# SonSang/dmesh_renderer

Measured on AMD Instinct MI355X. Metric: fwd+bwd Mpixels/sec @1080p, 500k tris; grad max-abs-err vs ref, higher is better.
Workload: dtype f32

## Files before the change

dmesh_renderer_amd/csrc/dmr_api.hip:

```cpp
#include <algorithm>
#include <atomic>
#include <chrono>
#include <cstdio>
#include <cstdlib>
#include <cstring>
#include <functional>
#include <map>
#include <mutex>
#include <string>
#include <vector>

#include "dmr_kernels.hpp"

namespace {

thread_local std::string g_err;

int fail(const std::string& m) { g_err = m; return 1; }

#define DMR_HIP(expr)                                                                           \
    do {                                                                                        \
        hipError_t e_ = (expr);                                                                 \
        if (e_ != hipSuccess) return fail(std::string(#expr) + ": " + hipGetErrorString(e_));   \
    } while (0)

constexpr size_t ALIGN = 256;
inline size_t up(size_t n) { return (n + ALIGN - 1) & ~(ALIGN - 1); }

struct Carver {
    char* base; size_t off;
    explicit Carver(void* b) : base(reinterpret_cast<char*>(b)), off(0) {}
    template <class T> T* take(size_t count) {
        T* p = base ? reinterpret_cast<T*>(base + off) : nullptr;
        off += up(count * sizeof(T));
        return p;
    }
};

struct PointState { float4* vproj; };
struct FaceState { uint2* rect; float* key_depth; float* max_depth; uint32_t* tiles_touched; void* facerec; void* colrec; void* tetrec; };
struct ImageState {
    uint32_t* tile_count; uint32_t* tile_offset; uint32_t* tile_cursor; int* num_rendered;
    float* final_T; float* final_prev_T; uint32_t* n_contrib;
    uint32_t* tile_hits; uint32_t* tile_bound; uint32_t* scan_tmp; uint32_t* hit_offset; uint32_t* tile_used; unsigned long long* hit_total; uint32_t* tile_order;
    int32_t* first_face; int32_t* first_tet; int32_t* last_face; int32_t* last_tet; uint8_t* is_active;
    float* mats;
    int* seed;
    unsigned long long* mask_offset;
    dmr::TetSeq* seq;
};
struct BinningState {
    uint64_t* keys; uint32_t* face_list; uint32_t capacity; unsigned long long mask_offset, mask_first;
    char* base; unsigned long long seq_offset; uint32_t seq_steps;
};

size_t carve_point(void* b, size_t BP, PointState& s) { Carver c(b); s.vproj = c.take<float4>(BP); return c.off; }
size_t carve_face(void* b, size_t BF, size_t F, size_t T, bool tet, FaceState& s) {
    Carver c(b);
    s.rect = c.take<uint2>(BF); s.key_depth = c.take<float>(BF);
    s.max_depth = tet ? c.take<float>(BF) : nullptr;
    s.tiles_touched = c.take<uint32_t>(BF);
    s.facerec = s.colrec = s.tetrec = nullptr;
    if (tet) {
        s.facerec = c.take<char>(F * dmr::tet_facerec_bytes());
        s.colrec = c.take<char>(F * dmr::tet_colrec_bytes());
        s.tetrec = c.take<char>(T * dmr::tet_tetrec_bytes());
    }
    return c.off;
}
size_t carve_image(void* b, size_t B, size_t ntiles, size_t npix, bool tet, ImageState& s) {
    Carver c(b);
    s.mats = c.take<float>(64 * B);
    s.seed = c.take<int>(1);
    s.mask_offset = c.take<unsigned long long>(2);
    s.tile_count = c.take<uint32_t>(ntiles); s.tile_hits = c.take<uint32_t>(ntiles); s.tile_bound = c.take<uint32_t>(ntiles);
    s.scan_tmp = c.take<uint32_t>(dmr::scan_tmp_words((int)ntiles));
    s.hit_offset = c.take<uint32_t>(ntiles + 1); s.tile_used = c.take<uint32_t>(ntiles); s.hit_total = c.take<unsigned long long>(1);
    s.tile_offset = c.take<uint32_t>(ntiles + 1);
    s.tile_cursor = c.take<uint32_t>(ntiles); s.num_rendered = c.take<int>(1);
    s.tile_order = c.take<uint32_t>(ntiles);
    s.final_T = c.take<float>(npix); s.final_prev_T = c.take<float>(npix); s.n_contrib = c.take<uint32_t>(npix);
    if (tet) {
        s.first_face = c.take<int32_t>(npix); s.first_tet = c.take<int32_t>(npix);
        s.last_face = c.take<int32_t>(npix); s.last_tet = c.take<int32_t>(npix);
        s.is_active = c.take<uint8_t>(npix);
        s.seq = c.take<dmr::TetSeq>(1);
    } else {
        s.first_face = s.first_tet = s.last_face = s.last_tet = nullptr; s.is_active = nullptr;
        s.seq = nullptr;
    }
    return c.off;
}
size_t carve_binning(void* b, size_t R, size_t mask_tiles, size_t seq_tiles, size_t seq_steps, BinningState& s) {
    Carver c(b);
    s.face_list = c.take<uint32_t>(R); s.keys = c.take<uint64_t>(R);
    s.capacity = (uint32_t)std::min<size_t>(R, 0xffffffffu);
    s.mask_offset = c.off;
    s.mask_first = dmr::mask_first_slots(R, mask_tiles);
    if (mask_tiles && R > 0) c.take<uint4>(dmr::mask_slots(R, mask_tiles) * 256);
    s.base = reinterpret_cast<char*>(b); s.seq_offset = c.off; s.seq_steps = (uint32_t)seq_steps;
    if (seq_steps) c.take<char>(dmr::tet_seq_bytes(seq_tiles, seq_steps));
    return c.off;
}

struct Dims { int gx, gy, r0, r1, ntiles; size_t BP, BF, npix; };

dmr_scene canonical(const dmr_scene* s, const float* mats) {
    dmr_scene c = *s;
    const size_t n = 16 * (size_t)s->B;
    c.mv_mats = mats; c.proj_mats = mats + n; c.inv_mv_mats = mats + 2 * n; c.inv_proj_mats = mats + 3 * n;
    c.mats_transposed = 0;
    return c;
}

int check_scene(const dmr_scene* s, bool tet, Dims& d) {
    if (!s) return fail("null scene");
    if (s->B <= 0 || s->W <= 0 || s->H <= 0 || s->P < 0 || s->F < 0 || s->T < 0) return fail("bad dimensions");
    if ((int64_t)s->B * s->P > INT32_MAX || (int64_t)s->B * s->F > INT32_MAX || (int64_t)s->B * s->W * s->H > INT32_MAX)
        return fail("problem too large for 32-bit indexing");
    d.gx = (s->W + dmr::TILE - 1) / dmr::TILE;
    d.gy = (s->H + dmr::TILE - 1) / dmr::TILE;
    if (d.gx > 65535 || d.gy > 65535) return fail("image too large (tile coordinates must fit 16 bits)");
    d.r0 = s->row_begin; d.r1 = s->row_end;
    if (d.r0 == 0 && d.r1 == 0) d.r1 = d.gy;
    d.r0 = std::max(0, std::min(d.gy, d.r0));
    d.r1 = std::max(d.r0, std::min(d.gy, d.r1));
    d.ntiles = s->B * d.gx * d.gy;
    d.BP = (size_t)s->B * s->P; d.BF = (size_t)s->B * s->F; d.npix = (size_t)s->B * s->W * s->H;
    if (tet && s->F > 0 && s->P > 0 && (!s->tets || !s->face_tets || !s->tet_faces)) return fail("tet topology missing");
    if (tet && s->F >= (1 << 28)) return fail("too many faces for the tet renderer (face ids must fit 28 bits)");
    return 0;
}

struct SizeRead {
    void* slot = nullptr; uint32_t seq = 0;
    volatile unsigned long long* word(int which) const { return reinterpret_cast<volatile unsigned long long*>(slot) + which; }
    uint32_t next_seq() { seq = (seq + 1u) & 0xffffffu; if (seq == 0u) seq = 1u; return seq; }
};
SizeRead* size_read() {
    thread_local std::map<int, SizeRead> per_device;
    int dev = 0;
    if (hipGetDevice(&dev) != hipSuccess) return nullptr;
    SizeRead& sr = per_device[dev];
    if (!sr.slot) {
        if (hipHostMalloc(&sr.slot, 64, hipHostMallocCoherent | hipHostMallocPortable) != hipSuccess) { sr.slot = nullptr; return nullptr; }
        memset(sr.slot, 0, 64);
    }
    return &sr;
}
int wait_size(volatile unsigned long long* w, uint32_t seq, hipStream_t st, unsigned long long* size) {
    const auto t0 = std::chrono::steady_clock::now();
    for (uint32_t spins = 0;; spins++) {
        const unsigned long long v = *w;
        if ((uint32_t)(v >> 40) == (seq & 0xffffffu)) { std::atomic_thread_fence(std::memory_order_acquire); *size = v & ((1ull << 40) - 1ull); return 0; }
        if ((spins & 1023u) == 1023u && std::chrono::steady_clock::now() - t0 > std::chrono::milliseconds(50)) break;
#if defined(__x86_64__) || defined(__i386__)
        __builtin_ia32_pause();
#endif
    }
    DMR_HIP(hipStreamSynchronize(st));
    const unsigned long long v = *w;
    if ((uint32_t)(v >> 40) != (seq & 0xffffffu)) return fail("the size word was not written (internal error)");
    *size = v & ((1ull << 40) - 1ull);
    return 0;
}

std::mutex g_overflow_mu;
std::map<int, uint32_t*> g_overflow;
uint32_t* overflow_word(int dev, bool create) {
    std::lock_guard<std::mutex> lk(g_overflow_mu);
    auto it = g_overflow.find(dev);
    if (it != g_overflow.end()) return it->second;
    if (!create) return nullptr;
    void* p = nullptr;
    if (hipHostMalloc(&p, 64, hipHostMallocCoherent | hipHostMallocPortable) != hipSuccess) return nullptr;
    *reinterpret_cast<volatile uint32_t*>(p) = 0u;
    return g_overflow[dev] = reinterpret_cast<uint32_t*>(p);
}

bool stream_is_capturing(hipStream_t st) {
    hipStreamCaptureStatus cs = hipStreamCaptureStatusNone;
    if (hipStreamIsCapturing(st, &cs) != hipSuccess) { (void)hipGetLastError(); return false; }
    return cs != hipStreamCaptureStatusNone;
}

struct SizeKey {
    int v[7];
    bool operator<(const SizeKey& o) const { return memcmp(v, o.v, sizeof(v)) < 0; }
};
struct SizeGuess { double rendered_per_face = 0.0, hits_per_face = 0.0; uint32_t* seq_steps = nullptr; };
std::mutex g_size_mu;
std::map<SizeKey, SizeGuess> g_size_cache;
std::atomic<uint64_t> g_redo_count{0};
int size_bucket(size_t BF) { int b = 0; while ((BF >> (b + 1)) != 0) b++; return b; }
SizeKey size_key(const dmr_scene* s, bool tet, const Dims& d) {
    return SizeKey{{s->B, s->W, s->H, d.r0, d.r1, tet ? 1 : 0, size_bucket(d.BF)}};
}
double lookup_estimate(const SizeKey& key, double SizeGuess::* field) {
    for (int db : {0, -1, 1}) {
        SizeKey k = key; k.v[6] += db;
        auto it = g_size_cache.find(k);
        if (it != g_size_cache.end() && it->second.*field > 0.0) return it->second.*field;
    }
    return 0.0;
}
uint64_t padded(uint64_t n) { return n + n / 4 + 4096; }

int run_forward(const dmr_scene* s, bool tet, const Dims& d, dmr_alloc_fn alloc, void* ctx, hipStream_t st,
                PointState& ps, FaceState& fs, ImageState& is, int* num_rendered,
                const std::function<void(const BinningState&)>& render) {
    PointState tp; FaceState tf; ImageState ti;
    void* pb = alloc(ctx, DMR_BUF_POINT, carve_point(nullptr, d.BP, tp));
    void* fb = alloc(ctx, DMR_BUF_FACE, carve_face(nullptr, d.BF, (size_t)s->F, (size_t)s->T, tet, tf));
    void* ib = alloc(ctx, DMR_BUF_IMAGE, carve_image(nullptr, (size_t)s->B, (size_t)d.ntiles, d.npix, tet, ti));
    if (!pb || !fb || !ib) return fail("scratch allocation failed");
    carve_point(pb, d.BP, ps);
    carve_face(fb, d.BF, (size_t)s->F, (size_t)s->T, tet, fs);
    carve_image(ib, (size_t)s->B, (size_t)d.ntiles, d.npix, tet, is);
    const bool async = (s->flags & DMR_FLAG_ASYNC) != 0 || stream_is_capturing(st);
    int dev = 0;
    DMR_HIP(hipGetDevice(&dev));
    uint32_t* overflow = overflow_word(dev, !async);

    auto front = [&](unsigned long long* host_R, uint32_t host_seq, uint64_t capacity, uint32_t* ovf) -> int {
        dmr::launch_project_verts(*s, ps.vproj, is.mats, is.tile_count, (size_t)(is.scan_tmp + dmr::SCAN_TMP_BUCKETS - is.tile_count), st);
        dmr::launch_setup_faces(*s, tet, ps.vproj, d.gx, d.gy, d.r0, d.r1, fs.rect, fs.key_depth, fs.max_depth,
                                fs.tiles_touched, is.tile_count, st);
        dmr::launch_scan_tiles(d.ntiles, is.tile_count, is.tile_offset, is.tile_cursor, is.num_rendered, host_R, host_seq, is.tile_order,
                               is.scan_tmp, (uint32_t)std::min<uint64_t>(capacity, 0xffffffffu), ovf, st);
        return 0;
    };
    size_t seq_steps = 0;
    if (tet) {
        std::lock_guard<std::mutex> lk(g_size_mu);
        SizeGuess& g = g_size_cache[size_key(s, tet, d)];
        if (!g.seq_steps && !async) {
            void* w = nullptr;
            if (hipHostMalloc(&w, 64, hipHostMallocCoherent | hipHostMallocPortable) == hipSuccess) {
                g.seq_steps = reinterpret_cast<uint32_t*>(w);
                *reinterpret_cast<volatile uint32_t*>(g.seq_steps) = 0u;
            } else (void)hipGetLastError();
        }
        if (g.seq_steps) {
            const uint64_t longest = *reinterpret_cast<volatile uint32_t*>(g.seq_steps);
            if (longest) {
                const uint64_t budget = 16ull << 30;
                const uint64_t per4 = dmr::tet_seq_bytes((size_t)d.ntiles, 4);
                seq_steps = (size_t)(std::min<uint64_t>((longest + longest / 4 + 4 + 3) / 4, std::max<uint64_t>(budget / std::max<uint64_t>(per4, 1), 1)) * 4);
            }
        }
    }
    auto rest = [&](uint64_t capacity) -> int {
        BinningState tb, bs;
        const size_t mask_tiles = tet ? 0 : (size_t)d.ntiles;
        void* bb = alloc(ctx, DMR_BUF_BINNING, carve_binning(nullptr, (size_t)capacity, mask_tiles, (size_t)d.ntiles, seq_steps, tb));
        if (!bb && (capacity > 0 || seq_steps > 0)) return fail("binning allocation failed");
        carve_binning(bb, (size_t)capacity, mask_tiles, (size_t)d.ntiles, seq_steps, bs);

        if (capacity > 0) {
            dmr::launch_scatter_faces(*s, d.gx, d.gy, fs.rect, fs.key_depth, fs.tiles_touched, is.tile_cursor, bs.keys,
                                      (uint32_t)capacity, tet ? nullptr : is.mask_offset, bs.mask_offset, bs.mask_first, st);
            if (d.ntiles > dmr::SCAN_SINGLE_MAX)
                dmr::launch_sort_tiles(d.ntiles, is.tile_offset, is.tile_order, bs.keys, bs.face_list, bs.capacity, st);
        }
        render(bs);
        return 0;
    };

    const SizeKey key = size_key(s, tet, d);
    uint64_t guess = 0;
    {
        std::lock_guard<std::mutex> lk(g_size_mu);
        const double per_face = lookup_estimate(key, &SizeGuess::rendered_per_face);
        if (per_face > 0.0) guess = std::min<uint64_t>(padded((uint64_t)(per_face * (double)d.BF)), 0x7fffffffu);
    }
    if (async) {
        if (!guess || !overflow)
            return fail("asynchronous / captured call without a size estimate: run one default (waiting) call with the same "
                        "view configuration first");
        if (front(nullptr, 0u, guess, overflow) || rest(guess)) return 1;
        *num_rendered = (int)guess;
        DMR_HIP(hipGetLastError());
        return 0;
    }
    SizeRead* sr = size_read();
    if (!sr) return fail("hipHostMalloc failed");
    const uint32_t seq = sr->next_seq();
    if (front(const_cast<unsigned long long*>(sr->word(0)), seq, ~0ull, nullptr)) return 1;
    if (guess && rest(guess)) return 1;
    unsigned long long R64 = 0;
    if (wait_size(sr->word(0), seq, st, &R64)) return 1;
    if (R64 > 0x7fffffffull) return fail("num_rendered overflows 31 bits");
    const int R = (int)R64;
    *num_rendered = R;
    if (!guess) {
        if (rest((uint64_t)R)) return 1;
    } else if ((uint64_t)R > guess) {
        g_redo_count.fetch_add(1, std::memory_order_relaxed);
        DMR_HIP(hipStreamSynchronize(st));
        if (front(nullptr, 0u, ~0ull, nullptr) || rest((uint64_t)R)) return 1;
    }
    {
        std::lock_guard<std::mutex> lk(g_size_mu);
        g_size_cache[key].rendered_per_face = (double)std::max(R, 1) / (double)std::max<size_t>(d.BF, 1);
    }
    DMR_HIP(hipGetLastError());
    return 0;
}

std::atomic<uint32_t> g_prof_mask{0};
struct ProfRec { int stage; hipEvent_t a, b; };
std::mutex g_prof_mu;
std::vector<ProfRec*> g_prof_live, g_prof_free;

}

namespace dmr {
StageScope::StageScope(int stage_, hipStream_t st_) : stage(stage_), st(st_), rec(nullptr) {
    if (!(g_prof_mask.load(std::memory_order_relaxed) & (1u << stage))) return;
    ProfRec* r = nullptr;
    {
        std::lock_guard<std::mutex> lk(g_prof_mu);
        if (!g_prof_free.empty()) { r = g_prof_free.back(); g_prof_free.pop_back(); }
    }
    if (!r) {
        r = new ProfRec();
        if (hipEventCreate(&r->a) != hipSuccess || hipEventCreate(&r->b) != hipSuccess) { delete r; return; }
    }
    r->stage = stage;
    (void)hipEventRecord(r->a, st);
    rec = r;
}
StageScope::~StageScope() {
    if (!rec) return;
    ProfRec* r = reinterpret_cast<ProfRec*>(rec);
    (void)hipEventRecord(r->b, st);
    std::lock_guard<std::mutex> lk(g_prof_mu);
    g_prof_live.push_back(r);
}
}

extern "C" {

void dmr_profile_enable(uint32_t mask) { g_prof_mask.store(mask); }

int dmr_profile_collect(double* ms, int64_t* launches) {
    std::vector<ProfRec*> live;
    {
        std::lock_guard<std::mutex> lk(g_prof_mu);
        live.swap(g_prof_live);
    }
    int rc = 0;
    for (ProfRec* r : live) {
        float t = 0.f;
        if (hipEventSynchronize(r->b) != hipSuccess || hipEventElapsedTime(&t, r->a, r->b) != hipSuccess) {
            g_err = "profile event read failed";
            rc = 1;
        } else if (r->stage >= 0 && r->stage < DMR_NUM_STAGES) {
            if (ms) ms[r->stage] += (double)t;
            if (launches) launches[r->stage] += 1;
        }
    }
    std::lock_guard<std::mutex> lk(g_prof_mu);
    for (ProfRec* r : live) g_prof_free.push_back(r);
    return rc;
}

const char* dmr_stage_name(int stage) {
    static const char* names[DMR_NUM_STAGES] = {"k_project_verts", "k_setup_faces", "k_scan_tiles", "k_scatter_faces",
                                                "k_sort_tiles", "k_tri_forward", "k_tri_backward_pix", "k_tri_unpack",
                                                "k_tet_first_intersect", "k_tet_forward", "k_tet_backward",
                                                "k_tri_backward_hits"};
    return (stage >= 0 && stage < DMR_NUM_STAGES) ? names[stage] : "?";
}

const char* dmr_last_error(void) { return g_err.c_str(); }

int dmr_overflowed(int device, int reset) {
    int dev = device;
    if (dev < 0 && hipGetDevice(&dev) != hipSuccess) return 0;
    uint32_t* w = overflow_word(dev, false);
    if (!w) return 0;
    volatile uint32_t* v = w;
    const int r = *v != 0u;
    if (reset) *v = 0u;
    return r;
}
uint64_t dmr_redo_count(void) { return g_redo_count.load(std::memory_order_relaxed); }
int dmr_abi_version(void) { return DMR_ABI_VERSION; }
const char* dmr_build_arch(void) { return "gfx950"; }

int dmr_tri_forward(const dmr_scene* s, float* out_color, float* out_depth, dmr_alloc_fn alloc, void* ctx,
                    void* stream, int* num_rendered) {
    Dims d;
    if (check_scene(s, false, d)) return 1;
    if (!alloc || !num_rendered || !out_color || !out_depth) return fail("null argument");
    *num_rendered = 0;
    if (s->P == 0 || s->F == 0) return 0;
    hipStream_t st = reinterpret_cast<hipStream_t>(stream);
    PointState ps; FaceState fs; ImageState is;
    auto render = [&](const BinningState& bs) {
        dmr::TriImageState img{is.final_T, is.final_prev_T, is.n_contrib, is.tile_hits, is.tile_bound, is.hit_offset, is.tile_used, is.tile_order, is.mask_offset};
        const dmr_scene sc = canonical(s, is.mats);
        dmr::launch_tri_forward(sc, d.gx, d.gy, d.r0, d.r1, ps.vproj, is.tile_offset, d.ntiles > dmr::SCAN_SINGLE_MAX ? nullptr : bs.keys,
                                bs.face_list, bs.capacity, img, out_color,
                                out_depth, st);
    };
    return run_forward(s, false, d, alloc, ctx, st, ps, fs, is, num_rendered, render);
}

int dmr_tri_backward(const dmr_scene* s, const float* dL_dcolor, const float* dL_ddepth, int num_rendered,
                     const void* point_buf, const void* face_buf, const void* binning_buf, const void* image_buf,
                     float* dL_dverts, float* dL_dvcolor, float* dL_dfopacity, float* dL_dvdepth, float* dL_dfintense,
                     dmr_alloc_fn alloc, void* ctx, void* stream) {
    Dims d;
    if (check_scene(s, false, d)) return 1;
    hipStream_t st = reinterpret_cast<hipStream_t>(stream);
    if (s->P == 0 || s->F == 0 || num_rendered <= 0 || d.r1 <= d.r0) {
        if (s->P > 0) {
            DMR_HIP(hipMemsetAsync(dL_dverts, 0, sizeof(float) * 3 * (size_t)s->P, st));
            DMR_HIP(hipMemsetAsync(dL_dvcolor, 0, sizeof(float) * 3 * (size_t)s->P, st));
            DMR_HIP(hipMemsetAsync(dL_dvdepth, 0, sizeof(float) * d.BP, st));
        }
        if (s->F > 0) {
            DMR_HIP(hipMemsetAsync(dL_dfopacity, 0, sizeof(float) * (size_t)s->F, st));
            DMR_HIP(hipMemsetAsync(dL_dfintense, 0, sizeof(float) * d.BF, st));
        }
        if (s->P > 0 && s->F > 0) {
            std::lock_guard<std::mutex> lk(g_size_mu);
            SizeGuess& g = g_size_cache[size_key(s, false, d)];
            if (!(g.hits_per_face > 0.0)) g.hits_per_face = 1.0 / (double)std::max<size_t>(d.BF, 1);
        }
        return 0;
    }
    if (!point_buf || !face_buf || !binning_buf || !image_buf || !alloc) return fail("null scratch buffer");
    PointState ps; FaceState fs; ImageState is; BinningState bs;
    carve_point(const_cast<void*>(point_buf), d.BP, ps);
    carve_face(const_cast<void*>(face_buf), d.BF, (size_t)s->F, (size_t)s->T, false, fs);
    carve_image(const_cast<void*>(image_buf), (size_t)s->B, (size_t)d.ntiles, d.npix, false, is);
    carve_binning(const_cast<void*>(binning_buf), (size_t)num_rendered, 0, 0, 0, bs);

    const bool async = (s->flags & DMR_FLAG_ASYNC) != 0 || stream_is_capturing(st);
    int dev = 0;
    DMR_HIP(hipGetDevice(&dev));
    uint32_t* overflow = overflow_word(dev, !async);
    const size_t vbytes = up(sizeof(float) * dmr::VROW * d.BP), fbytes = up(sizeof(float) * dmr::FROW * d.BF);
    const size_t pbytes = up(sizeof(float4) * 2 * (size_t)d.ntiles * dmr::TILE_PIX);
    auto rest = [&](uint64_t capacity, dmr::HitRegions regions) -> int {
        const size_t hbytes = up(sizeof(dmr::HitRecord) * (size_t)capacity);
        char* work = reinterpret_cast<char*>(alloc(ctx, DMR_BUF_WORK, vbytes + fbytes + pbytes + hbytes));
        if (!work) return fail("workspace allocation failed");
        float* vrow = reinterpret_cast<float*>(work);
        float* frow = reinterpret_cast<float*>(work + vbytes);
        float4* pixrec = reinterpret_cast<float4*>(work + vbytes + fbytes);
        dmr::HitRecord* hits = reinterpret_cast<dmr::HitRecord*>(work + vbytes + fbytes + pbytes);
        dmr::TriImageState img{is.final_T, is.final_prev_T, is.n_contrib, is.tile_hits, is.tile_bound, is.hit_offset, is.tile_used, is.tile_order, is.mask_offset};
        const dmr_scene sc = canonical(s, is.mats);
        dmr::launch_tri_backward_pix(sc, d.gx, d.gy, d.r0, d.r1, ps.vproj, is.tile_offset, bs.face_list, img,
                                     dL_dcolor, dL_ddepth, pixrec, hits, (uint32_t)capacity,
                                     reinterpret_cast<float*>(work), (vbytes + fbytes) / sizeof(float), regions, st);
        dmr::launch_tri_backward_hits(sc, d.gx, d.gy, ps.vproj, bs.face_list, img, pixrec, hits, (uint32_t)capacity, vrow, frow, st);
        dmr::launch_tri_unpack(*s, vrow, frow, dL_dverts, dL_dvcolor, dL_dfopacity, dL_dvdepth, dL_dfintense, st);
        return 0;
    };
    const dmr::HitRegions scanned{nullptr, nullptr, nullptr, nullptr, 0u};
    const bool self_regions = d.ntiles <= dmr::SCAN_SINGLE_MAX;
    const SizeKey key = size_key(s, false, d);
    uint64_t guess = 0;
    {
        std::lock_guard<std::mutex> lk(g_size_mu);
        const double per_face = lookup_estimate(key, &SizeGuess::hits_per_face);
        if (per_face > 0.0) guess = std::min<uint64_t>(padded((uint64_t)(per_face * (double)d.BF)), 0xfffffffeull);
    }
    if (async) {
        if (!guess || !overflow)
            return fail("asynchronous / captured call without a size estimate: run one default (waiting) backward with the "
                        "same view configuration first");
        if (self_regions) {
            if (rest(guess, dmr::HitRegions{is.hit_offset, is.hit_total, nullptr, overflow, 0u})) return 1;
        } else {
            dmr::launch_scan_hits(d.ntiles, is.tile_hits, is.tile_offset, is.hit_offset, is.tile_used, is.hit_total, nullptr, 0u, is.scan_tmp, (uint32_t)guess, overflow, st);
            if (rest(guess, scanned)) return 1;
        }
        DMR_HIP(hipGetLastError());
        return 0;
    }
    SizeRead* sr = size_read();
    if (!sr) return fail("hipHostMalloc failed");
    unsigned long long* host_total = const_cast<unsigned long long*>(sr->word(1));
    const uint32_t seq = sr->next_seq();
    if (guess && self_regions) {
        if (rest(guess, dmr::HitRegions{is.hit_offset, is.hit_total, host_total, nullptr, seq})) return 1;
    } else {
        dmr::launch_scan_hits(d.ntiles, is.tile_hits, is.tile_offset, is.hit_offset, is.tile_used, is.hit_total, host_total, seq, is.scan_tmp, 0xffffffffu, nullptr, st);
        if (guess && rest(guess, scanned)) return 1;
    }
    unsigned long long nhits = 0;
    if (wait_size(sr->word(1), seq, st, &nhits)) return 1;
    if (nhits >= 0xffffffffull) return fail("more than 2^32 blended (pixel, face) pairs");
    if (!guess) {
        if (rest(nhits, scanned)) return 1;
    } else if (nhits > guess) {
        g_redo_count.fetch_add(1, std::memory_order_relaxed);
        DMR_HIP(hipStreamSynchronize(st));
        if (self_regions) {
            if (rest(nhits, dmr::HitRegions{is.hit_offset, is.hit_total, nullptr, nullptr, 0u})) return 1;
        } else if (rest(nhits, scanned)) return 1;
    }
    {
        std::lock_guard<std::mutex> lk(g_size_mu);
        g_size_cache[key].hits_per_face = (double)std::max<uint64_t>(nhits, 1) / (double)std::max<size_t>(d.BF, 1);
    }
    DMR_HIP(hipGetLastError());
    return 0;
}

int dmr_tet_forward(const dmr_scene* s, float* out_color, float* out_depth, float* out_active, dmr_alloc_fn alloc,
                    void* ctx, void* stream, int* num_rendered) {
    Dims d;
    if (check_scene(s, true, d)) return 1;
    if (!alloc || !num_rendered || !out_color || !out_depth || !out_active) return fail("null argument");
    *num_rendered = 0;
    hipStream_t st = reinterpret_cast<hipStream_t>(stream);
    PointState ps; FaceState fs; ImageState is;
    auto render = [&](const BinningState& bs) {
        dmr::TetImageState img{is.final_T, is.final_prev_T, is.n_contrib, is.first_face, is.first_tet,
                               is.last_face, is.last_tet, is.is_active, fs.facerec, fs.colrec, fs.tetrec, is.seed,
                               is.seq, bs.base};
        const dmr_scene sc = canonical(s, is.mats);
        dmr::launch_tet_prep(sc, img, bs.seq_steps, bs.seq_offset, st);
        dmr::launch_tet_first_intersect(sc, d.gx, d.gy, d.r0, d.r1, fs.key_depth, fs.max_depth, is.tile_offset,
                                        d.ntiles > dmr::SCAN_SINGLE_MAX ? nullptr : bs.keys, bs.face_list, bs.capacity, img, st);
        dmr::launch_tet_forward(sc, d.gx, d.gy, d.r0, d.r1, img, out_color, out_depth, out_active, st);
    };
    return run_forward(s, true, d, alloc, ctx, st, ps, fs, is, num_rendered, render);
}

int dmr_tet_backward(const dmr_scene* s, const float* dL_dcolor, const float* dL_ddepth, const void* point_buf,
                     const void* face_buf, const void* binning_buf, const void* image_buf, float* dL_dvcolor,
                     float* dL_dfopacity, dmr_alloc_fn alloc, void* ctx, void* stream) {
    Dims d;
    if (check_scene(s, true, d)) return 1;
    hipStream_t st = reinterpret_cast<hipStream_t>(stream);
    float* full = nullptr;
    if ((s->flags & DMR_FLAG_TET_FULL_GRADS) && 3 * (int64_t)s->P + (int64_t)d.BF > 0) {
        if (!alloc) return fail("null argument");
        const int64_t n = 3 * (int64_t)s->P + (int64_t)d.BF;
        full = static_cast<float*>(alloc(ctx, DMR_BUF_TET_GRADS, (size_t)n * sizeof(float)));
        if (!full) return fail("allocation of the tet gradient buffer failed");
        dmr::launch_tet_zero_grads(full, 3 * (int64_t)s->P, full + 3 * (int64_t)s->P, (int64_t)d.BF, st);
    }
    dmr::launch_tet_zero_grads(dL_dvcolor, 3 * (int64_t)s->P, dL_dfopacity, (int64_t)s->F, st);
    if (s->P == 0 || s->F == 0) return 0;
    if (!image_buf || !face_buf) return fail("null scratch buffer");
    ImageState is; FaceState fs;
    carve_image(const_cast<void*>(image_buf), (size_t)s->B, (size_t)d.ntiles, d.npix, true, is);
    carve_face(const_cast<void*>(face_buf), d.BF, (size_t)s->F, (size_t)s->T, true, fs);
    dmr::TetImageState img{is.final_T, is.final_prev_T, is.n_contrib, is.first_face, is.first_tet,
                           is.last_face, is.last_tet, is.is_active, fs.facerec, fs.colrec, fs.tetrec, is.seed,
                           is.seq, reinterpret_cast<char*>(const_cast<void*>(binning_buf))};
    const dmr_scene sc = canonical(s, is.mats);
    uint32_t* host_seq_steps = nullptr;
    {
        std::lock_guard<std::mutex> lk(g_size_mu);
        auto it = g_size_cache.find(size_key(s, true, d));
        if (it != g_size_cache.end()) host_seq_steps = it->second.seq_steps;
    }
    dmr::launch_tet_backward(sc, d.gx, d.gy, d.r0, d.r1, img, dL_dcolor, dL_ddepth, dL_dvcolor, dL_dfopacity, host_seq_steps, st,
                             full, full ? full + 3 * (int64_t)s->P : nullptr);
    DMR_HIP(hipGetLastError());
    return 0;
}

namespace {
__global__ void k_invert_mats(const float* __restrict__ in, int count, int transposed, float* __restrict__ out) {
    const int m = blockIdx.x * blockDim.x + threadIdx.x;
    if (m >= count) return;
    double a[16];
#pragma unroll
    for (int k = 0; k < 16; k++) a[k] = (double)in[16 * m + (transposed ? 4 * (k & 3) + (k >> 2) : k)];
    const double s0 = a[0] * a[5] - a[1] * a[4], s1 = a[0] * a[6] - a[2] * a[4], s2 = a[0] * a[7] - a[3] * a[4];
    const double s3 = a[1] * a[6] - a[2] * a[5], s4 = a[1] * a[7] - a[3] * a[5], s5 = a[2] * a[7] - a[3] * a[6];
    const double c5 = a[10] * a[15] - a[11] * a[14], c4 = a[9] * a[15] - a[11] * a[13], c3 = a[9] * a[14] - a[10] * a[13];
    const double c2 = a[8] * a[15] - a[11] * a[12], c1 = a[8] * a[14] - a[10] * a[12], c0 = a[8] * a[13] - a[9] * a[12];
    const double det = s0 * c5 - s1 * c4 + s2 * c3 + s3 * c2 - s4 * c1 + s5 * c0;
    const double r = 1.0 / det;
    double b[16];
    b[0] = (a[5] * c5 - a[6] * c4 + a[7] * c3) * r;   b[1] = (-a[1] * c5 + a[2] * c4 - a[3] * c3) * r;
    b[2] = (a[13] * s5 - a[14] * s4 + a[15] * s3) * r; b[3] = (-a[9] * s5 + a[10] * s4 - a[11] * s3) * r;
    b[4] = (-a[4] * c5 + a[6] * c2 - a[7] * c1) * r;  b[5] = (a[0] * c5 - a[2] * c2 + a[3] * c1) * r;
    b[6] = (-a[12] * s5 + a[14] * s2 - a[15] * s1) * r; b[7] = (a[8] * s5 - a[10] * s2 + a[11] * s1) * r;
    b[8] = (a[4] * c4 - a[5] * c2 + a[7] * c0) * r;   b[9] = (-a[0] * c4 + a[1] * c2 - a[3] * c0) * r;
    b[10] = (a[12] * s4 - a[13] * s2 + a[15] * s0) * r; b[11] = (-a[8] * s4 + a[9] * s2 - a[11] * s0) * r;
    b[12] = (-a[4] * c3 + a[5] * c1 - a[6] * c0) * r; b[13] = (a[0] * c3 - a[1] * c1 + a[2] * c0) * r;
    b[14] = (-a[12] * s3 + a[13] * s1 - a[14] * s0) * r; b[15] = (a[8] * s3 - a[9] * s1 + a[10] * s0) * r;
#pragma unroll
    for (int k = 0; k < 16; k++) out[16 * m + k] = (float)b[k];
}
}

int dmr_invert_mats(const float* in, int count, int transposed, float* out, void* stream) {
    if (count < 0 || (count > 0 && (!in || !out))) return fail("dmr_invert_mats: bad arguments");
    if (count == 0) return 0;
    hipStream_t st = reinterpret_cast<hipStream_t>(stream);
    k_invert_mats<<<dim3((unsigned)((count + 63) / 64)), dim3(64), 0, st>>>(in, count, transposed, out);
    DMR_HIP(hipGetLastError());
    return 0;
}

namespace {
__global__ void k_export_vproj(const float4* v, int64_t n, int what, float* dst) {
    const int64_t i = (int64_t)blockIdx.x * blockDim.x + threadIdx.x;
    if (i >= n) return;
    if (what == 0) { dst[2 * i] = v[i].x; dst[2 * i + 1] = v[i].y; }
    else dst[i] = v[i].z;
}
__global__ void k_export_ranges(const uint32_t* off, const uint32_t* cnt, int64_t n, uint32_t* dst) {
    const int64_t i = (int64_t)blockIdx.x * blockDim.x + threadIdx.x;
    if (i >= n) return;
    const bool empty = cnt[i] == 0;
    dst[2 * i] = empty ? 0u : off[i];
    dst[2 * i + 1] = empty ? 0u : off[i + 1];
}
}

int64_t dmr_export(const dmr_scene* s, int is_tet, int num_rendered, const char* name, const void* point_buf,
                   const void* face_buf, const void* binning_buf, const void* image_buf, void* dst, int64_t cap,
                   void* stream) {
    Dims d;
    if (!name || check_scene(s, is_tet != 0, d)) return -1;
    hipStream_t st = reinterpret_cast<hipStream_t>(stream);
    PointState ps; FaceState fs; ImageState is; BinningState bs;
    carve_point(const_cast<void*>(point_buf), d.BP, ps);
    carve_face(const_cast<void*>(face_buf), d.BF, (size_t)s->F, (size_t)s->T, is_tet != 0, fs);
    carve_image(const_cast<void*>(image_buf), (size_t)s->B, (size_t)d.ntiles, d.npix, is_tet != 0, is);
    carve_binning(const_cast<void*>(binning_buf), (size_t)std::max(0, num_rendered), 0, 0, 0, bs);
    const std::string n(name);
    auto plain = [&](const void* src, size_t bytes) -> int64_t {
        if (dst && src && bytes) {
            if (hipMemcpyAsync(dst, src, std::min<size_t>(bytes, (size_t)cap), hipMemcpyDeviceToDevice, st) != hipSuccess) {
                g_err = "export copy failed";
                return -1;
            }
        }
        return (int64_t)bytes;
    };
    if (n == "image" || n == "ndc_z") {
        const size_t bytes = d.BP * (n == "image" ? 8 : 4);
        if (dst && d.BP && (size_t)cap >= bytes)
            k_export_vproj<<<dim3((unsigned)((d.BP + 255) / 256)), dim3(256), 0, st>>>(
                ps.vproj, (int64_t)d.BP, n == "image" ? 0 : 1, reinterpret_cast<float*>(dst));
        return (int64_t)bytes;
    }
    if (n == "ranges") {
        const size_t bytes = (size_t)d.ntiles * 8;
        if (dst && (size_t)cap >= bytes)
            k_export_ranges<<<dim3((unsigned)((d.ntiles + 255) / 256)), dim3(256), 0, st>>>(
                is.tile_offset, is.tile_count, d.ntiles, reinterpret_cast<uint32_t*>(dst));
        return (int64_t)bytes;
    }
    if (n == "key_depth") return plain(fs.key_depth, d.BF * 4);
    if (n == "max_depth") return is_tet ? plain(fs.max_depth, d.BF * 4) : -1;
    if (n == "tiles_touched") return plain(fs.tiles_touched, d.BF * 4);
    if (n == "face_list") return plain(bs.face_list, (size_t)std::max(0, num_rendered) * 4);
    if (n == "final_T") return plain(is.final_T, d.npix * 4);
    if (n == "final_prev_T") return plain(is.final_prev_T, d.npix * 4);
    if (n == "n_contrib") return plain(is.n_contrib, d.npix * 4);
    if (n == "tile_hits") return is_tet ? -1 : plain(is.tile_hits, (size_t)d.ntiles * 4);
    if (is_tet) {
        if (n == "first_face") return plain(is.first_face, d.npix * 4);
        if (n == "first_tet") return plain(is.first_tet, d.npix * 4);
        if (n == "last_face") return plain(is.last_face, d.npix * 4);
        if (n == "last_tet") return plain(is.last_tet, d.npix * 4);
        if (n == "is_active") return plain(is.is_active, d.npix);
        if (n == "tet_seq") return plain(is.seq, 8);
    }
    g_err = "unknown export item: " + n;
    return -1;
}

}
```

dmesh_renderer_amd/csrc/dmr_binning.hip:

```cpp
#include <algorithm>

#include "dmr_kernels.hpp"
#include "dmr_sort.hpp"

namespace dmr {

__device__ __forceinline__ float mat_at(const float* __restrict__ m, int k, bool transposed) {
    return m[transposed ? 4 * (k & 3) + (k >> 2) : k];
}

__global__ void __launch_bounds__(256)
k_project_verts(int B, int P, const float* __restrict__ verts, const float* __restrict__ mv_mats,
                const float* __restrict__ proj_mats, const float* __restrict__ inv_mv_mats,
                const float* __restrict__ inv_proj_mats, int transposed, const float* __restrict__ verts_depth,
                int W, int H, float4* __restrict__ vproj, float* __restrict__ mats,
                uint32_t* __restrict__ counters, uint32_t ncounters) {
    {
        const uint32_t per = (ncounters + gridDim.x - 1) / gridDim.x;
        const uint32_t z0 = min(ncounters, blockIdx.x * per), z1 = min(ncounters, z0 + per);
        for (uint32_t i = z0 + threadIdx.x; i < z1; i += 256) counters[i] = 0u;
    }
    if (blockIdx.x == 0) {
        for (int i = threadIdx.x; i < 64 * B; i += 256) {
            const int m = i / (16 * B), r = i % (16 * B);
            const float* src = m == 0 ? mv_mats : (m == 1 ? proj_mats : (m == 2 ? inv_mv_mats : inv_proj_mats));
            mats[i] = mat_at(src + 16 * (r >> 4), r & 15, (transposed >> m) & 1);
        }
    }
    const int64_t idx = (int64_t)blockIdx.x * blockDim.x + threadIdx.x;
    if (idx >= (int64_t)B * P) return;
    const int b = (int)(idx / P), p = (int)(idx % P);
    float mv[16], pr[16];
#pragma unroll
    for (int k = 0; k < 16; k++) {
        mv[k] = mat_at(mv_mats + 16 * b, k, transposed & 1);
        pr[k] = mat_at(proj_mats + 16 * b, k, (transposed >> 1) & 1);
    }
    V3 pv = xform4x3(load_v3(verts, p), mv);
    V4 pc = xform4x4(pv, pr);
    float p_w = (float)(1.0 / (double)clamp_w(pc.w));
    V3 n = {pc.x * p_w, pc.y * p_w, pc.z * p_w};
    vproj[idx] = make_float4(ndc2pix(n.x, W), ndc2pix(n.y, H), n.z, verts_depth[idx]);
}

constexpr int LDS_HIST_MAX = 8192;
__host__ inline int bin_fpt(int64_t n) { return n < 256 * 1024 ? 1 : n < 1024 * 1024 ? 2 : 4; }
constexpr uint32_t BIG_RECT = 256;

struct BinWindow { int x0, y0, wx, wy, view; bool lds; };

constexpr int BIG_MAX = 128;
struct BigFace { uint32_t rect_lo, rect_hi, tile_base, key_lo, key_hi; };

struct RectWalk {
    uint32_t w, n, i, x, y, dx, dy;
    __device__ __forceinline__ RectWalk(uint32_t minx, uint32_t miny, uint32_t maxx, uint32_t maxy, uint32_t tid) {
        w = maxx - minx; n = w * (maxy - miny); i = tid;
        y = miny + tid / w; x = minx + tid % w; dy = 256u / w; dx = 256u % w;
        x0 = minx;
    }
    uint32_t x0;
    __device__ __forceinline__ bool valid() const { return i < n; }
    __device__ __forceinline__ void next() {
        i += 256u; y += dy; x += dx;
        if (x >= x0 + w) { x -= w; y++; }
    }
};

template <int FPT>
__device__ __forceinline__ BinWindow bin_window(int* s_box, int view, const uint2* rr, const uint32_t* touched,
                                                const bool* mine, int tid) {
    int bx0 = 0x7fffffff, by0 = 0x7fffffff, bx1 = 0, by1 = 0;
#pragma unroll
    for (int it = 0; it < FPT; it++) {
        if (!mine[it] || touched[it] == 0 || touched[it] > BIG_RECT) continue;
        bx0 = min(bx0, (int)(rr[it].x & 0xffffu)); by0 = min(by0, (int)(rr[it].x >> 16));
        bx1 = max(bx1, (int)(rr[it].y & 0xffffu)); by1 = max(by1, (int)(rr[it].y >> 16));
    }
#pragma unroll
    for (int d = 32; d > 0; d >>= 1) {
        bx0 = min(bx0, __shfl_xor(bx0, d, 64)); by0 = min(by0, __shfl_xor(by0, d, 64));
        bx1 = max(bx1, __shfl_xor(bx1, d, 64)); by1 = max(by1, __shfl_xor(by1, d, 64));
    }
    if (tid == 0) { s_box[0] = 0x7fffffff; s_box[1] = 0x7fffffff; s_box[2] = 0; s_box[3] = 0; }
    __syncthreads();
    if ((tid & 63) == 0) {
        atomicMin(&s_box[0], bx0); atomicMin(&s_box[1], by0); atomicMax(&s_box[2], bx1); atomicMax(&s_box[3], by1);
    }
    __syncthreads();
    BinWindow w;
    w.x0 = s_box[0]; w.y0 = s_box[1]; w.wx = s_box[2] - s_box[0]; w.wy = s_box[3] - s_box[1]; w.view = view;
    w.lds = w.wx > 0 && w.wy > 0 && (int64_t)w.wx * w.wy <= LDS_HIST_MAX;
    if (!w.lds) { w.wx = 0; w.wy = 0; }
    return w;
}

template <bool TET, int FPT>
__global__ void __launch_bounds__(256)
k_setup_faces_lds(int B, int P, int F, const int* __restrict__ faces, const float4* __restrict__ vproj,
                  int gx, int gy, int r0, int r1,
                  uint2* __restrict__ face_rect, float* __restrict__ key_depth, float* __restrict__ max_depth,
                  uint32_t* __restrict__ tiles_touched, uint32_t* __restrict__ tile_count) {
    __shared__ uint32_t s_hist[LDS_HIST_MAX];
    __shared__ int s_box[4];
    __shared__ BigFace s_big[BIG_MAX];
    __shared__ uint32_t s_nbig;
    const int tid = threadIdx.x;
    if (tid == 0) s_nbig = 0u;
    const int64_t BF = (int64_t)B * F;
    const int64_t base = (int64_t)blockIdx.x * (256 * FPT);
    const int view = (int)(base / F);
    uint2 rr[FPT];
    uint32_t touched[FPT];
    bool mine[FPT];
#pragma unroll
    for (int it = 0; it < FPT; it++) {
        const int64_t idx = base + it * 256 + tid;
        touched[it] = 0u; rr[it] = make_uint2(0, 0); mine[it] = false;
        if (idx >= BF) continue;
        const int b = (int)(idx / F), f = (int)(idx % F);
        mine[it] = b == view;
        const int v0 = faces[3 * f], v1 = faces[3 * f + 1], v2 = faces[3 * f + 2];
        const float4 a0 = vproj[(int64_t)b * P + v0], a1 = vproj[(int64_t)b * P + v1], a2 = vproj[(int64_t)b * P + v2];
        float max_z = a0.z, min_z = a0.z, depth = 0.0f;
        depth += a0.z;
        max_z = fmaxf(max_z, a1.z); min_z = fminf(min_z, a1.z); depth += a1.z;
        max_z = fmaxf(max_z, a2.z); min_z = fminf(min_z, a2.z); depth += a2.z;
        depth = depth / 3.0f;
        Rect r = {0, 0, 0, 0};
        if (!(max_z < -1.0f || min_z > 1.0f)) {
            r = tile_rect({a0.x, a0.y}, {a1.x, a1.y}, {a2.x, a2.y}, gx, gy, r0, r1);
            touched[it] = (r.maxy - r.miny) * (r.maxx - r.minx);
        }
        if (touched[it] == 0) r = {0, 0, 0, 0};
        auto map01 = [](float z) { float d = (z + 1.0f) * 0.5f; if (d < 0.0f) d = 0.0f; if (d > 1.0f) d = 1.0f; return d; };
        rr[it] = make_uint2(r.minx | (r.miny << 16), r.maxx | (r.maxy << 16));
        tiles_touched[idx] = touched[it];
        face_rect[idx] = rr[it];
        key_depth[idx] = touched[it] ? (TET ? map01(min_z) : map01(depth)) : 0.0f;
        if (TET) max_depth[idx] = touched[it] ? map01(max_z) : 0.0f;
    }
    const BinWindow w = bin_window<FPT>(s_box, view, rr, touched, mine, tid);
    const int nw = w.wx * w.wy;
    for (int t = tid; t < nw; t += 256) s_hist[t] = 0u;
    __syncthreads();
#pragma unroll
    for (int it = 0; it < FPT; it++) {
        if (touched[it] == 0) continue;
        const int64_t idx = base + it * 256 + tid;
        const uint32_t tb = (uint32_t)(idx / F) * gx * gy;
        const uint32_t minx = rr[it].x & 0xffffu, miny = rr[it].x >> 16, maxx = rr[it].y & 0xffffu, maxy = rr[it].y >> 16;
        if (touched[it] > BIG_RECT) {
            const uint32_t q = atomicAdd(&s_nbig, 1u);
            if (q < (uint32_t)BIG_MAX) { s_big[q] = BigFace{rr[it].x, rr[it].y, tb, 0u, 0u}; continue; }
        }
        if (w.lds && mine[it] && touched[it] <= BIG_RECT) {
            for (uint32_t y = miny; y < maxy; y++)
                for (uint32_t x = minx; x < maxx; x++) atomicAdd(&s_hist[(y - w.y0) * w.wx + (x - w.x0)], 1u);
        } else {
            for (uint32_t y = miny; y < maxy; y++)
                for (uint32_t x = minx; x < maxx; x++) atomicAdd(&tile_count[tb + y * gx + x], 1u);
        }
    }
    __syncthreads();
    for (int y = tid / 64; y < w.wy; y += 4)
        for (int x = tid % 64; x < w.wx; x += 64) {
            const uint32_t c = s_hist[y * w.wx + x];
            if (c) atomicAdd(&tile_count[(uint32_t)view * gx * gy + (uint32_t)(w.y0 + y) * gx + (uint32_t)(w.x0 + x)], c);
        }
    const uint32_t nbig = min(s_nbig, (uint32_t)BIG_MAX);
    for (uint32_t q = 0; q < nbig; q++) {
        const BigFace f = s_big[q];
        for (RectWalk t(f.rect_lo & 0xffffu, f.rect_lo >> 16, f.rect_hi & 0xffffu, f.rect_hi >> 16, (uint32_t)tid); t.valid(); t.next())
            atomicAdd(&tile_count[f.tile_base + t.y * gx + t.x], 1u);
    }
}

template <int FPT>
__global__ void __launch_bounds__(256)
k_scatter_faces_lds(int B, int F, int gx, int gy, const uint2* __restrict__ face_rect,
                    const float* __restrict__ key_depth, const uint32_t* __restrict__ tiles_touched,
                    uint32_t* __restrict__ tile_cursor, uint64_t* __restrict__ keys, uint32_t capacity,
                    unsigned long long* __restrict__ mask_offset_dst, unsigned long long mask_offset, unsigned long long mask_first) {
    if (mask_offset_dst && blockIdx.x == 0 && threadIdx.x == 0) { mask_offset_dst[0] = mask_offset; mask_offset_dst[1] = mask_first; }
    __shared__ uint32_t s_hist[LDS_HIST_MAX];
    __shared__ int s_box[4];
    __shared__ BigFace s_big[BIG_MAX];
    __shared__ uint32_t s_nbig;
    const int tid = threadIdx.x;
    if (tid == 0) s_nbig = 0u;
    const int64_t BF = (int64_t)B * F;
    const int64_t base = (int64_t)blockIdx.x * (256 * FPT);
    const int view = (int)(base / F);
    uint2 rr[FPT];
    uint32_t touched[FPT];
    bool mine[FPT];
#pragma unroll
    for (int it = 0; it < FPT; it++) {
        const int64_t idx = base + it * 256 + tid;
        touched[it] = idx < BF ? tiles_touched[idx] : 0u;
        rr[it] = touched[it] ? face_rect[idx] : make_uint2(0, 0);
        mine[it] = idx < BF && (int)(idx / F) == view;
    }
    const BinWindow w = bin_window<FPT>(s_box, view, rr, touched, mine, tid);
    const int nw = w.wx * w.wy;
    for (int t = tid; t < nw; t += 256) s_hist[t] = 0u;
    __syncthreads();
#pragma unroll
    for (int it = 0; it < FPT; it++) {
        if (!(w.lds && mine[it]) || touched[it] == 0 || touched[it] > BIG_RECT) continue;
        const uint32_t minx = rr[it].x & 0xffffu, miny = rr[it].x >> 16, maxx = rr[it].y & 0xffffu, maxy = rr[it].y >> 16;
        for (uint32_t y = miny; y < maxy; y++)
            for (uint32_t x = minx; x < maxx; x++) atomicAdd(&s_hist[(y - w.y0) * w.wx + (x - w.x0)], 1u);
    }
    __syncthreads();
    for (int y = tid / 64; y < w.wy; y += 4)
        for (int x = tid % 64; x < w.wx; x += 64) {
            const uint32_t c = s_hist[y * w.wx + x];
            if (c) s_hist[y * w.wx + x] = atomicAdd(&tile_cursor[(uint32_t)view * gx * gy + (uint32_t)(w.y0 + y) * gx + (uint32_t)(w.x0 + x)], c);
        }
    __syncthreads();
#pragma unroll
    for (int it = 0; it < FPT; it++) {
        if (touched[it] == 0) continue;
        const int64_t idx = base + it * 256 + tid;
        const int f = (int)(idx % F);
        const uint32_t tb = (uint32_t)(idx / F) * gx * gy;
        const uint32_t minx = rr[it].x & 0xffffu, miny = rr[it].x >> 16, maxx = rr[it].y & 0xffffu, maxy = rr[it].y >> 16;
        const uint64_t key = ((uint64_t)__float_as_uint(key_depth[idx]) << 32) | (uint32_t)f;
        if (touched[it] > BIG_RECT) {
            const uint32_t q = atomicAdd(&s_nbig, 1u);
            if (q < (uint32_t)BIG_MAX) { s_big[q] = BigFace{rr[it].x, rr[it].y, tb, (uint32_t)key, (uint32_t)(key >> 32)}; continue; }
        }
        const bool direct = !(w.lds && mine[it]) || touched[it] > BIG_RECT;
        for (uint32_t y = miny; y < maxy; y++)
            for (uint32_t x = minx; x < maxx; x++) {
                const uint32_t slot = direct ? atomicAdd(&tile_cursor[tb + y * gx + x], 1u)
                                             : atomicAdd(&s_hist[(y - w.y0) * w.wx + (x - w.x0)], 1u);
                if (slot < capacity) keys[slot] = key;
            }
    }
    __syncthreads();
    const uint32_t nbig = min(s_nbig, (uint32_t)BIG_MAX);
    for (uint32_t q = 0; q < nbig; q++) {
        const BigFace f = s_big[q];
        const uint64_t key = ((uint64_t)f.key_hi << 32) | f.key_lo;
        for (RectWalk t(f.rect_lo & 0xffffu, f.rect_lo >> 16, f.rect_hi & 0xffffu, f.rect_hi >> 16, (uint32_t)tid); t.valid();) {
            uint32_t tile[4], slot[4];
#pragma unroll
            for (int u = 0; u < 4; u++) {
                tile[u] = 0xffffffffu;
                if (t.valid()) { tile[u] = f.tile_base + t.y * gx + t.x; t.next(); }
            }
#pragma unroll
            for (int u = 0; u < 4; u++) slot[u] = tile[u] != 0xffffffffu ? atomicAdd(&tile_cursor[tile[u]], 1u) : 0xffffffffu;
#pragma unroll
            for (int u = 0; u < 4; u++) if (slot[u] < capacity) keys[slot[u]] = key;
        }
    }
}

constexpr int ORDER_BUCKETS = 64;
__device__ __forceinline__ int order_bucket(uint32_t n) { return ORDER_BUCKETS - 1 - (int)min(n >> 4, (uint32_t)(ORDER_BUCKETS - 1)); }
constexpr int ORDER_COPIES = 16;
constexpr int ORDER_CELLS = ORDER_BUCKETS * ORDER_COPIES;
__device__ __forceinline__ int order_cell(uint32_t n, int lane) { return order_bucket(n) * ORDER_COPIES + (lane & (ORDER_COPIES - 1)); }

constexpr int SCAN_BATCH = 8;

__device__ __forceinline__ uint32_t block_exclusive_scan(uint32_t local, int tid, uint32_t* wave_sum ) {
    const int lane = tid & 63, wave = tid >> 6;
    uint32_t incl = local;
#pragma unroll
    for (int d = 1; d < 64; d <<= 1) {
        uint32_t o = __shfl_up(incl, d, 64);
        if (lane >= d) incl += o;
    }
    if (lane == 63) wave_sum[wave] = incl;
    __syncthreads();
    if (tid < 64) {
        const uint32_t w = tid < 16 ? wave_sum[tid] : 0u;
        uint32_t wi = w;
#pragma unroll
        for (int d = 1; d < 16; d <<= 1) {
            uint32_t o = __shfl_up(wi, d, 64);
            if (tid >= d) wi += o;
        }
        if (tid < 16) wave_sum[tid] = wi - w;
        if (tid == 15) wave_sum[16] = wi;
    }
    __syncthreads();
    return wave_sum[wave] + incl - local;
}

constexpr int SCAN_SLAB = 1024 * SCAN_BATCH;

__device__ __forceinline__ void slab_load(uint32_t* __restrict__ slab, const uint32_t* __restrict__ src, int n, int tid) {
#pragma unroll
    for (int j = 0; j < SCAN_BATCH; j++) { const int i = j * 1024 + tid; slab[i] = i < n ? src[i] : 0u; }
}
__device__ __forceinline__ void slab_read(const uint32_t* __restrict__ slab, int tid, uint32_t (&c)[SCAN_BATCH]) {
    static_assert(SCAN_BATCH == 8, "two 16-byte LDS reads per thread");
    const uint4 lo = *reinterpret_cast<const uint4*>(slab + tid * SCAN_BATCH), hi = *reinterpret_cast<const uint4*>(slab + tid * SCAN_BATCH + 4);
    c[0] = lo.x; c[1] = lo.y; c[2] = lo.z; c[3] = lo.w; c[4] = hi.x; c[5] = hi.y; c[6] = hi.z; c[7] = hi.w;
}
__device__ __forceinline__ void slab_write_offsets(uint32_t* __restrict__ slab, int tid, uint32_t run, const uint32_t (&c)[SCAN_BATCH]) {
    uint32_t o[SCAN_BATCH];
#pragma unroll
    for (int j = 0; j < SCAN_BATCH; j++) { o[j] = run; run += c[j]; }
    *reinterpret_cast<uint4*>(slab + tid * SCAN_BATCH) = make_uint4(o[0], o[1], o[2], o[3]);
    *reinterpret_cast<uint4*>(slab + tid * SCAN_BATCH + 4) = make_uint4(o[4], o[5], o[6], o[7]);
}

__global__ void __launch_bounds__(1024)
k_scan_tiles(int n, const uint32_t* __restrict__ tile_count, uint32_t* __restrict__ tile_offset,
             uint32_t* __restrict__ tile_cursor, int* __restrict__ num_rendered, unsigned long long* __restrict__ host_num_rendered,
             uint32_t host_seq, uint32_t* __restrict__ tile_order, uint32_t capacity, uint32_t* __restrict__ overflow) {
    static_assert(ORDER_CELLS == 1024, "one counter cell per thread");
    __shared__ uint32_t wave_sum[17];
    __shared__ uint32_t bucket[ORDER_CELLS + 1];
    __shared__ __attribute__((aligned(16))) uint32_t slab[SCAN_SLAB];
    const int tid = threadIdx.x, lane = tid & 63;
    const int begin = tid * SCAN_BATCH;
    bucket[tid] = 0u;
    slab_load(slab, tile_count, n, tid);
    __syncthreads();
    uint32_t c[SCAN_BATCH], local = 0;
    slab_read(slab, tid, c);
#pragma unroll
    for (int j = 0; j < SCAN_BATCH; j++) {
        local += c[j];
        if (c[j]) atomicAdd(&bucket[order_cell(c[j], lane)], 1u);
    }
    const uint32_t run = block_exclusive_scan(local, tid, wave_sum);
    const uint32_t total = wave_sum[16];
    slab_write_offsets(slab, tid, run, c);
    __syncthreads();
    const uint32_t cell_base = block_exclusive_scan(bucket[tid], tid, wave_sum);
    bucket[tid] = cell_base;
    if (tid == 0) bucket[ORDER_CELLS] = wave_sum[16];
#pragma unroll
    for (int j = 0; j < SCAN_BATCH; j++) {
        const int i = j * 1024 + tid;
        if (i < n) { const uint32_t o = slab[i]; tile_offset[i] = o; tile_cursor[i] = o; }
    }
    __syncthreads();
#pragma unroll
    for (int j = 0; j < SCAN_BATCH; j++) {
        const bool in = begin + j < n;
        const bool empty = in && c[j] == 0u;
        const uint64_t em = __ballot(empty);
        uint32_t ebase = 0;
        if (em) {
            const int leader = __ffsll((long long)em) - 1;
            if (lane == leader) ebase = atomicAdd(&bucket[ORDER_CELLS], (uint32_t)__popcll(em));
            ebase = __shfl(ebase, leader, 64);
        }
        if (empty) slab[ebase + (uint32_t)__popcll(em & ((1ull << lane) - 1ull))] = (uint32_t)(begin + j);
        else if (in) slab[atomicAdd(&bucket[order_cell(c[j], lane)], 1u)] = (uint32_t)(begin + j);
    }
    __syncthreads();
#pragma unroll
    for (int j = 0; j < SCAN_BATCH; j++) { const int i = j * 1024 + tid; if (i < n) tile_order[i] = slab[i]; }
    if (tid == 0) {
        tile_offset[n] = total; *num_rendered = (int)total;
        if (host_num_rendered) *host_num_rendered = host_size_word(host_seq, total);
        if (overflow && total > capacity) *overflow = 1u;
    }
}


constexpr int SCAN_BLOCK_TILES = 8192;
static_assert(SCAN_SINGLE_MAX == SCAN_SLAB, "up to here one workgroup does it all (k_scan_tiles, k_scan_hits)");

template <bool ORDER>
__global__ void __launch_bounds__(1024)
k_scan_tiles_partial(int n, const uint32_t* __restrict__ tile_count, const uint32_t* __restrict__ len_offset, uint32_t* __restrict__ blk_sum,
                     uint32_t* __restrict__ bucket_count) {
    __shared__ uint32_t wave_sum[17];
    __shared__ uint32_t bucket[ORDER_CELLS];
    const int tid = threadIdx.x, lane = tid & 63;
    const int begin = min(n, (int)blockIdx.x * SCAN_BLOCK_TILES + tid * SCAN_BATCH), end = min(n, begin + SCAN_BATCH);
    if (ORDER) bucket[tid] = 0u;
    __syncthreads();
    uint32_t c[SCAN_BATCH], local = 0;
#pragma unroll
    for (int j = 0; j < SCAN_BATCH; j++) {
        c[j] = begin + j < end ? tile_count[begin + j] : 0u;
        if (!ORDER && begin + j < end) c[j] = record_bound(c[j], len_offset[begin + j + 1] - len_offset[begin + j]);
    }
#pragma unroll
    for (int j = 0; j < SCAN_BATCH; j++) {
        local += c[j];
        if (ORDER && begin + j < end && c[j]) atomicAdd(&bucket[order_cell(c[j], lane)], 1u);
    }
    block_exclusive_scan(local, tid, wave_sum);
    if (tid == 0) blk_sum[blockIdx.x] = wave_sum[16];
    if (ORDER && tid < ORDER_BUCKETS) {
        uint32_t cnt = 0;
#pragma unroll
        for (int q = 0; q < ORDER_COPIES; q++) cnt += bucket[tid * ORDER_COPIES + q];
        if (cnt) atomicAdd(&bucket_count[tid], cnt);
    }
}

__global__ void __launch_bounds__(1024)
k_scan_tiles_blocks(int nblk, int n, uint32_t* __restrict__ blk_sum, uint32_t* __restrict__ bucket_count,
                    uint32_t* __restrict__ tile_offset, int* __restrict__ num_rendered, unsigned long long* __restrict__ host_num_rendered,
                    unsigned long long* __restrict__ total64, unsigned long long* __restrict__ host_total64, uint32_t host_seq,
                    uint32_t capacity, uint32_t* __restrict__ overflow) {
    __shared__ uint32_t wave_sum[17];
    const int tid = threadIdx.x, lane = tid & 63;
    unsigned long long carry = 0;
    for (int i0 = 0; i0 < nblk; i0 += 1024) {
        const uint32_t v = i0 + tid < nblk ? blk_sum[i0 + tid] : 0u;
        const uint32_t ex = block_exclusive_scan(v, tid, wave_sum);
        if (i0 + tid < nblk) blk_sum[i0 + tid] = (uint32_t)carry + ex;
        carry += wave_sum[16];
        __syncthreads();
    }
    if (tid == 0) {
        tile_offset[n] = (uint32_t)carry;
        if (num_rendered) { *num_rendered = (int)carry; if (host_num_rendered) *host_num_rendered = host_size_word(host_seq, carry); }
        if (total64) { *total64 = carry; if (host_total64) *host_total64 = host_size_word(host_seq, carry); }
        if (overflow && carry > (unsigned long long)capacity) *overflow = 1u;
    }
    if (bucket_count && tid < 128) {
        const uint32_t c = tid < ORDER_BUCKETS ? bucket_count[tid] : 0u;
        uint32_t bi = c;
#pragma unroll
        for (int d = 1; d < 64; d <<= 1) {
            uint32_t o = __shfl_up(bi, d, 64);
            if (lane >= d) bi += o;
        }
        if (tid < ORDER_BUCKETS) bucket_count[tid] = bi - c;
        if (tid == ORDER_BUCKETS - 1) bucket_count[ORDER_BUCKETS] = bi;
    }
}

template <bool ORDER>
__global__ void __launch_bounds__(1024)
k_scan_tiles_final(int n, const uint32_t* __restrict__ tile_count, const uint32_t* __restrict__ len_offset, const uint32_t* __restrict__ blk_sum,
                   uint32_t* __restrict__ bucket_cursor, uint32_t* __restrict__ tile_offset, uint32_t* __restrict__ tile_cursor,
                   uint32_t* __restrict__ tile_order) {
    __shared__ uint32_t wave_sum[17];
    __shared__ uint32_t bucket[ORDER_CELLS + 1];
    const int tid = threadIdx.x, lane = tid & 63;
    const int begin = min(n, (int)blockIdx.x * SCAN_BLOCK_TILES + tid * SCAN_BATCH), end = min(n, begin + SCAN_BATCH);
    if (ORDER) { bucket[tid] = 0u; if (tid == 0) bucket[ORDER_CELLS] = 0u; }
    __syncthreads();
    uint32_t c[SCAN_BATCH], local = 0;
    int n_empty = 0;
#pragma unroll
    for (int j = 0; j < SCAN_BATCH; j++) {
        c[j] = begin + j < end ? tile_count[begin + j] : 0u;
        if (!ORDER && begin + j < end) {
            c[j] = record_bound(c[j], len_offset[begin + j + 1] - len_offset[begin + j]);
            tile_cursor[begin + j] = 0u;
        }
    }
#pragma unroll
    for (int j = 0; j < SCAN_BATCH; j++) {
        local += c[j];
        if (ORDER && begin + j < end) {
            if (c[j]) atomicAdd(&bucket[order_cell(c[j], lane)], 1u);
            else n_empty++;
        }
    }
    if (ORDER) {
#pragma unroll
        for (int d = 32; d > 0; d >>= 1) n_empty += __shfl_xor(n_empty, d, 64);
        if (lane == 0 && n_empty) atomicAdd(&bucket[ORDER_CELLS], (uint32_t)n_empty);
    }
    uint32_t run = blk_sum[blockIdx.x] + block_exclusive_scan(local, tid, wave_sum);
    if (ORDER && tid < ORDER_BUCKETS) {
        uint32_t cnt = 0;
#pragma unroll
        for (int q = 0; q < ORDER_COPIES; q++) cnt += bucket[tid * ORDER_COPIES + q];
        uint32_t base = cnt ? atomicAdd(&bucket_cursor[tid], cnt) : 0u;
#pragma unroll
        for (int q = 0; q < ORDER_COPIES; q++) { const uint32_t k = bucket[tid * ORDER_COPIES + q]; bucket[tid * ORDER_COPIES + q] = base; base += k; }
    }
    if (ORDER && tid == ORDER_BUCKETS) { const uint32_t cnt = bucket[ORDER_CELLS]; bucket[ORDER_CELLS] = cnt ? atomicAdd(&bucket_cursor[ORDER_BUCKETS], cnt) : 0u; }
    __syncthreads();
#pragma unroll
    for (int j = 0; j < SCAN_BATCH; j++) {
        const bool in = begin + j < end;
        if (in) { tile_offset[begin + j] = run; if (ORDER) tile_cursor[begin + j] = run; }
        run += c[j];
        if (!ORDER) continue;
        const bool empty = in && c[j] == 0u;
        const uint64_t em = __ballot(empty);
        uint32_t ebase = 0;
        if (em) {
            const int leader = __ffsll((long long)em) - 1;
            if (lane == leader) ebase = atomicAdd(&bucket[ORDER_CELLS], (uint32_t)__popcll(em));
            ebase = __shfl(ebase, leader, 64);
        }
        if (empty) tile_order[ebase + (uint32_t)__popcll(em & ((1ull << lane) - 1ull))] = (uint32_t)(begin + j);
        else if (in) tile_order[atomicAdd(&bucket[order_cell(c[j], lane)], 1u)] = (uint32_t)(begin + j);
    }
}

__global__ void __launch_bounds__(1024)
k_scan_hits(int n, const uint32_t* __restrict__ tile_hits, const uint32_t* __restrict__ tile_offset, uint32_t* __restrict__ hit_offset,
            uint32_t* __restrict__ tile_used, unsigned long long* __restrict__ hit_total, unsigned long long* __restrict__ host_hit_total, uint32_t host_seq,
            uint32_t capacity, uint32_t* __restrict__ overflow) {
    __shared__ uint32_t wave_sum[17];
    __shared__ unsigned long long s_total;
    __shared__ __attribute__((aligned(16))) uint32_t slab[SCAN_SLAB];
    const int tid = threadIdx.x, lane = tid & 63;
    if (tid == 0) s_total = 0ull;
#pragma unroll
    for (int j = 0; j < SCAN_BATCH; j++) {
        const int i = j * 1024 + tid;
        slab[i] = i < n ? record_bound(tile_hits[i], tile_offset[i + 1] - tile_offset[i]) : 0u;
        if (i < n) tile_used[i] = 0u;
    }
    __syncthreads();
    uint32_t c[SCAN_BATCH], local = 0;
    slab_read(slab, tid, c);
    unsigned long long wide = 0;
#pragma unroll
    for (int j = 0; j < SCAN_BATCH; j++) { local += c[j]; wide += c[j]; }
#pragma unroll
    for (int d = 32; d > 0; d >>= 1) wide += __shfl_xor(wide, d, 64);
    const uint32_t run = block_exclusive_scan(local, tid, wave_sum);
    if (lane == 0) atomicAdd(&s_total, wide);
    slab_write_offsets(slab, tid, run, c);
    __syncthreads();
#pragma unroll
    for (int j = 0; j < SCAN_BATCH; j++) { const int i = j * 1024 + tid; if (i < n) hit_offset[i] = slab[i]; }
    if (tid == 0) {
        hit_offset[n] = wave_sum[16]; *hit_total = s_total;
        if (host_hit_total) *host_hit_total = host_size_word(host_seq, s_total);
        if (overflow && s_total > (unsigned long long)capacity) *overflow = 1u;
    }
}

__global__ void __launch_bounds__(256)
k_sort_tiles(uint32_t ntiles, const uint32_t* __restrict__ tile_offset, const uint32_t* __restrict__ tile_order,
             uint64_t* __restrict__ keys, uint32_t* __restrict__ face_list, uint32_t capacity) {
    __shared__ uint64_t s_keys[SORT_LDS_KEYS];
    __shared__ uint32_t s_rank[SORT_LDS_KEYS];
    for (uint32_t ti = blockIdx.x; ti < ntiles; ti += gridDim.x) {
        const uint32_t tile = tile_order[ti];
        const uint32_t begin = tile_offset[tile], end = tile_offset[tile + 1];
        if (end == begin || end > capacity) continue;
        __syncthreads();
        sort_tile(begin, end - begin, keys, face_list, s_keys, s_rank, threadIdx.x);
    }
}

void launch_project_verts(const dmr_scene& s, float4* vproj, float* mats, uint32_t* counters, size_t ncounters,
                          hipStream_t st) {
    const int64_t n = (int64_t)s.B * s.P;
    StageScope t(DMR_STAGE_PROJECT, st);
    k_project_verts<<<dim3((unsigned)std::max<int64_t>(1, (n + 255) / 256)), dim3(256), 0, st>>>(
        s.B, s.P, s.verts, s.mv_mats, s.proj_mats, s.inv_mv_mats, s.inv_proj_mats, s.mats_transposed, s.verts_depth,
        s.W, s.H, vproj, mats, counters, (uint32_t)ncounters);
}

void launch_setup_faces(const dmr_scene& s, bool tet, const float4* vproj, int gx, int gy, int r0, int r1,
                        uint2* face_rect, float* key_depth, float* max_depth, uint32_t* tiles_touched,
                        uint32_t* tile_count, hipStream_t st) {
    const int64_t n = (int64_t)s.B * s.F;
    if (n == 0) return;
    StageScope t(DMR_STAGE_SETUP_FACES, st);
    const int fpt = bin_fpt(n);
    dim3 grid((unsigned)((n + 256 * fpt - 1) / (256 * fpt))), block(256);
#define DMR_SETUP(TET, FPT) k_setup_faces_lds<TET, FPT><<<grid, block, 0, st>>>(s.B, s.P, s.F, s.faces, vproj, gx, gy, r0, r1, \
                                face_rect, key_depth, max_depth, tiles_touched, tile_count)
    if (tet) { if (fpt == 1) DMR_SETUP(true, 1); else if (fpt == 2) DMR_SETUP(true, 2); else DMR_SETUP(true, 4); }
    else { if (fpt == 1) DMR_SETUP(false, 1); else if (fpt == 2) DMR_SETUP(false, 2); else DMR_SETUP(false, 4); }
#undef DMR_SETUP
}

void launch_scan_tiles(int ntiles, const uint32_t* tile_count, uint32_t* tile_offset, uint32_t* tile_cursor,
                       int* num_rendered, unsigned long long* host_num_rendered, uint32_t host_seq, uint32_t* tile_order, uint32_t* scan_tmp,
                       uint32_t capacity, uint32_t* overflow, hipStream_t st) {
    StageScope t(DMR_STAGE_SCAN, st);
    if (ntiles <= SCAN_SINGLE_MAX) {
        k_scan_tiles<<<dim3(1), dim3(1024), 0, st>>>(ntiles, tile_count, tile_offset, tile_cursor, num_rendered, host_num_rendered, host_seq, tile_order,
                                                    capacity, overflow);
        return;
    }
    const int nblk = (ntiles + SCAN_BLOCK_TILES - 1) / SCAN_BLOCK_TILES;
    uint32_t* bucket = scan_tmp;
    uint32_t* blk_sum = scan_tmp + SCAN_TMP_BUCKETS;
    k_scan_tiles_partial<true><<<dim3(nblk), dim3(1024), 0, st>>>(ntiles, tile_count, nullptr, blk_sum, bucket);
    k_scan_tiles_blocks<<<dim3(1), dim3(1024), 0, st>>>(nblk, ntiles, blk_sum, bucket, tile_offset, num_rendered, host_num_rendered,
                                                        nullptr, nullptr, host_seq, capacity, overflow);
    k_scan_tiles_final<true><<<dim3(nblk), dim3(1024), 0, st>>>(ntiles, tile_count, nullptr, blk_sum, bucket, tile_offset, tile_cursor, tile_order);
}

size_t scan_tmp_words(int ntiles) { return SCAN_TMP_BUCKETS + (size_t)(ntiles + SCAN_BLOCK_TILES - 1) / SCAN_BLOCK_TILES + 1; }

void launch_scan_hits(int ntiles, const uint32_t* tile_hits, const uint32_t* tile_offset, uint32_t* hit_offset, uint32_t* tile_used,
                      unsigned long long* hit_total, unsigned long long* host_hit_total, uint32_t host_seq, uint32_t* scan_tmp, uint32_t capacity,
                      uint32_t* overflow, hipStream_t st) {
    StageScope t(DMR_STAGE_SCAN, st);
    if (ntiles <= SCAN_SINGLE_MAX) {
        k_scan_hits<<<dim3(1), dim3(1024), 0, st>>>(ntiles, tile_hits, tile_offset, hit_offset, tile_used, hit_total, host_hit_total, host_seq, capacity, overflow);
        return;
    }
    const int nblk = (ntiles + SCAN_BLOCK_TILES - 1) / SCAN_BLOCK_TILES;
    uint32_t* blk_sum = scan_tmp + SCAN_TMP_BUCKETS;
    k_scan_tiles_partial<false><<<dim3(nblk), dim3(1024), 0, st>>>(ntiles, tile_hits, tile_offset, blk_sum, nullptr);
    k_scan_tiles_blocks<<<dim3(1), dim3(1024), 0, st>>>(nblk, ntiles, blk_sum, nullptr, hit_offset, nullptr, nullptr, hit_total,
                                                        host_hit_total, host_seq, capacity, overflow);
    k_scan_tiles_final<false><<<dim3(nblk), dim3(1024), 0, st>>>(ntiles, tile_hits, tile_offset, blk_sum, nullptr, hit_offset, tile_used, nullptr);
}

void launch_scatter_faces(const dmr_scene& s, int gx, int gy, const uint2* face_rect, const float* key_depth,
                          const uint32_t* tiles_touched, uint32_t* tile_cursor, uint64_t* keys, uint32_t capacity,
                          unsigned long long* mask_offset_dst, unsigned long long mask_offset, unsigned long long mask_first, hipStream_t st) {
    const int64_t n = (int64_t)s.B * s.F;
    if (n == 0) return;
    StageScope t(DMR_STAGE_SCATTER, st);
    const int fpt = bin_fpt(n);
    const dim3 grid((unsigned)((n + 256 * fpt - 1) / (256 * fpt))), block(256);
#define DMR_SCATTER(FPT) k_scatter_faces_lds<FPT><<<grid, block, 0, st>>>(s.B, s.F, gx, gy, face_rect, key_depth, tiles_touched, \
                                                                         tile_cursor, keys, capacity, mask_offset_dst, mask_offset, mask_first)
    if (fpt == 1) DMR_SCATTER(1); else if (fpt == 2) DMR_SCATTER(2); else DMR_SCATTER(4);
#undef DMR_SCATTER
}

void launch_sort_tiles(int ntiles, const uint32_t* tile_offset, const uint32_t* tile_order, uint64_t* keys,
                       uint32_t* face_list, uint32_t capacity, hipStream_t st) {
    if (ntiles == 0) return;
    StageScope t(DMR_STAGE_SORT, st);
    k_sort_tiles<<<dim3((unsigned)std::min(ntiles, 256 * 64)), dim3(256), 0, st>>>((uint32_t)ntiles, tile_offset, tile_order, keys, face_list, capacity);
}

}
```

dmesh_renderer_amd/csrc/dmr_kernels.hpp:

```cpp
#pragma once

#include <hip/hip_runtime.h>
#include <stdint.h>

#include "../../include/dmesh_renderer_amd.h"
#include "dmr_device.hpp"

namespace dmr {

constexpr int VROW = 8;
constexpr int FROW = 2;
constexpr int HIT_GROUP = 4;
constexpr int HIT_BLOCK = 64 * HIT_GROUP;
__host__ __device__ inline uint32_t hit_slot_address(uint32_t rel) {
    return (rel & ~(uint32_t)(HIT_BLOCK - 1)) + (rel & (uint32_t)(HIT_GROUP - 1)) * 64u + ((rel & (uint32_t)(HIT_BLOCK - 1)) / (uint32_t)HIT_GROUP);
}

__host__ __device__ inline uint32_t record_bound(uint32_t h, uint32_t len) {
    if (h == 0u) return 0u;
    const uint32_t b = h + (uint32_t)(HIT_GROUP - 1) * (len < h ? len : h);
    return (b + (uint32_t)(HIT_BLOCK - 1)) & ~(uint32_t)(HIT_BLOCK - 1);
}
constexpr int SCAN_SINGLE_MAX = 8192;

struct StageScope {
    int stage; hipStream_t st; void* rec;
    StageScope(int stage, hipStream_t st);
    ~StageScope();
};

void launch_project_verts(const dmr_scene& s, float4* vproj, float* mats, uint32_t* counters, size_t ncounters,
                          hipStream_t st);
void launch_setup_faces(const dmr_scene& s, bool tet, const float4* vproj, int gx, int gy, int r0, int r1,
                        uint2* face_rect, float* key_depth, float* max_depth, uint32_t* tiles_touched,
                        uint32_t* tile_count, hipStream_t st);
constexpr int SCAN_TMP_BUCKETS = 128;
size_t scan_tmp_words(int ntiles);
__host__ __device__ inline unsigned long long host_size_word(uint32_t seq, unsigned long long size) {
    return ((unsigned long long)(seq & 0xffffffu) << 40) | (size < (1ull << 40) ? size : (1ull << 40) - 1ull);
}
void launch_scan_tiles(int ntiles, const uint32_t* tile_count, uint32_t* tile_offset, uint32_t* tile_cursor,
                       int* num_rendered, unsigned long long* host_num_rendered, uint32_t host_seq, uint32_t* tile_order, uint32_t* scan_tmp,
                       uint32_t capacity, uint32_t* overflow, hipStream_t st);
void launch_scatter_faces(const dmr_scene& s, int gx, int gy, const uint2* face_rect, const float* key_depth,
                          const uint32_t* tiles_touched, uint32_t* tile_cursor, uint64_t* keys, uint32_t capacity,
                          unsigned long long* mask_offset_dst, unsigned long long mask_offset, unsigned long long mask_first, hipStream_t st);
void launch_sort_tiles(int ntiles, const uint32_t* tile_offset, const uint32_t* tile_order, uint64_t* keys,
                       uint32_t* face_list, uint32_t capacity, hipStream_t st);

struct TriImageState {
    float* final_T; float* final_prev_T; uint32_t* n_contrib;
    uint32_t* tile_hits;
    uint32_t* tile_bound;
    const uint32_t* hit_offset;
    uint32_t* tile_used;
    const uint32_t* tile_order;
    const unsigned long long* mask_offset;
};
constexpr int MASK_CHUNK = 128;
inline size_t mask_first_slots(size_t list_capacity, size_t ntiles) { return list_capacity < ntiles ? list_capacity : ntiles; }
inline size_t mask_slots(size_t list_capacity, size_t ntiles) { return mask_first_slots(list_capacity, ntiles) + list_capacity / MASK_CHUNK + 1; }
struct alignas(16) HitRecord { uint32_t id; uint32_t pixel; float T; float dL_dalpha; };
void launch_tri_forward(const dmr_scene& s, int gx, int gy, int r0, int r1, const float4* vproj,
                        const uint32_t* tile_offset, uint64_t* keys, uint32_t* face_list, uint32_t capacity, TriImageState img,
                        float* out_color, float* out_depth, hipStream_t st);
void launch_scan_hits(int ntiles, const uint32_t* tile_hits, const uint32_t* tile_offset, uint32_t* hit_offset, uint32_t* tile_used,
                      unsigned long long* hit_total, unsigned long long* host_hit_total, uint32_t host_seq, uint32_t* scan_tmp, uint32_t capacity,
                      uint32_t* overflow, hipStream_t st);
struct HitRegions {
    uint32_t* hit_offset;
    unsigned long long* hit_total; unsigned long long* host_hit_total; uint32_t* overflow;
    uint32_t host_seq;
};
void launch_tri_backward_pix(const dmr_scene& s, int gx, int gy, int r0, int r1, const float4* vproj,
                             const uint32_t* tile_offset, const uint32_t* face_list, TriImageState img,
                             const float* dL_dcolor, const float* dL_ddepth, float4* pixrec, HitRecord* hits,
                             uint32_t capacity, float* work, size_t work_floats, HitRegions regions, hipStream_t st);
void launch_tri_backward_hits(const dmr_scene& s, int gx, int gy, const float4* vproj, const uint32_t* face_list, TriImageState img,
                              const float4* pixrec, const HitRecord* hits, uint32_t capacity, float* vrow, float* frow,
                              hipStream_t st);
void launch_tri_unpack(const dmr_scene& s, const float* vrow, const float* frow, float* dL_dverts,
                       float* dL_dvcolor, float* dL_dfopacity, float* dL_dvdepth, float* dL_dfintense,
                       hipStream_t st);

struct TetSeq {
    uint32_t max_steps;
    uint32_t cap_steps;
    unsigned long long offset;
};
inline size_t tet_seq_bytes(size_t ntiles, size_t cap_steps) { return ntiles * 4 * (cap_steps / 4) * 1024; }
struct TetImageState {
    float* final_log_T; float* final_prev_log_T; uint32_t* n_contrib;
    int32_t* first_face; int32_t* first_tet; int32_t* last_face; int32_t* last_tet; uint8_t* is_active;
    void* facerec; void* colrec; void* tetrec;
    int* seed;
    TetSeq* seq;
    char* binning;
};
size_t tet_facerec_bytes();
size_t tet_colrec_bytes();
size_t tet_tetrec_bytes();
void launch_tet_prep(const dmr_scene& s, TetImageState img, uint32_t seq_steps, unsigned long long seq_offset, hipStream_t st);
void launch_tet_first_intersect(const dmr_scene& s, int gx, int gy, int r0, int r1, const float* key_depth,
                                const float* max_depth, const uint32_t* tile_offset, uint64_t* keys, uint32_t* face_list,
                                uint32_t capacity, TetImageState img, hipStream_t st);
void launch_tet_forward(const dmr_scene& s, int gx, int gy, int r0, int r1, TetImageState img,
                        float* out_color, float* out_depth, float* out_active, hipStream_t st);
void launch_tet_zero_grads(float* dL_dvcolor, int64_t n_vcolor, float* dL_dfopacity, int64_t n_fopacity, hipStream_t st);
void launch_tet_backward(const dmr_scene& s, int gx, int gy, int r0, int r1, TetImageState img,
                         const float* dL_dcolor, const float* dL_ddepth, float* dL_dvcolor, float* dL_dfopacity,
                         uint32_t* host_seq_steps, hipStream_t st, float* dL_dverts = nullptr, float* dL_dfintense = nullptr);

}
```

Measured before the change: 7112.

## Fuse tile scan into scatter kernel with cursor-relative slots and chunked decoupled scan

Folds the tile prefix scan into the scatter launch. Extra workgroups scan tile-count chunks and publish the results through a global sync area, while the face workgroups reserve per-tile counts relative to a zeroed cursor before waiting for the offsets. Slots become tile_offset plus the cursor value, so scatter no longer has to wait for a separate scan kernel, which removes one launch and its serialization. The cost is inter-workgroup spin-waits that rely on forward progress, guarded by a bounded-wait timeout flag that invalidates the call, plus more counter words to zero.

```diff
diff --git a/dmesh_renderer_amd/csrc/dmr_api.hip b/dmesh_renderer_amd/csrc/dmr_api.hip
--- a/dmesh_renderer_amd/csrc/dmr_api.hip
+++ b/dmesh_renderer_amd/csrc/dmr_api.hip
@@ -42,7 +42,7 @@
 struct ImageState {
     uint32_t* tile_count; uint32_t* tile_offset; uint32_t* tile_cursor; int* num_rendered;
     float* final_T; float* final_prev_T; uint32_t* n_contrib;
-    uint32_t* tile_hits; uint32_t* tile_bound; uint32_t* scan_tmp; uint32_t* hit_offset; uint32_t* tile_used; unsigned long long* hit_total; uint32_t* tile_order;
+    uint32_t* tile_hits; uint32_t* tile_bound; uint32_t* scan_tmp; uint32_t* fuse_sync; uint32_t* hit_offset; uint32_t* tile_used; unsigned long long* hit_total; uint32_t* tile_order;
     int32_t* first_face; int32_t* first_tet; int32_t* last_face; int32_t* last_tet; uint8_t* is_active;
     float* mats;
     int* seed;
@@ -74,10 +74,12 @@
     s.seed = c.take<int>(1);
     s.mask_offset = c.take<unsigned long long>(2);
     s.tile_count = c.take<uint32_t>(ntiles); s.tile_hits = c.take<uint32_t>(ntiles); s.tile_bound = c.take<uint32_t>(ntiles);
+    s.tile_cursor = c.take<uint32_t>(ntiles);
     s.scan_tmp = c.take<uint32_t>(dmr::scan_tmp_words((int)ntiles));
+    s.fuse_sync = c.take<uint32_t>(dmr::fuse_sync_words((int)ntiles));
     s.hit_offset = c.take<uint32_t>(ntiles + 1); s.tile_used = c.take<uint32_t>(ntiles); s.hit_total = c.take<unsigned long long>(1);
     s.tile_offset = c.take<uint32_t>(ntiles + 1);
-    s.tile_cursor = c.take<uint32_t>(ntiles); s.num_rendered = c.take<int>(1);
+    s.num_rendered = c.take<int>(1);
     s.tile_order = c.take<uint32_t>(ntiles);
     s.final_T = c.take<float>(npix); s.final_prev_T = c.take<float>(npix); s.n_contrib = c.take<uint32_t>(npix);
     if (tet) {
@@ -91,6 +93,7 @@
     }
     return c.off;
 }
+size_t counters_words(const ImageState& s, int ntiles) { return (size_t)(s.fuse_sync + dmr::fuse_sync_words(ntiles) - s.tile_count); }
 size_t carve_binning(void* b, size_t R, size_t mask_tiles, size_t seq_tiles, size_t seq_steps, BinningState& s) {
     Carver c(b);
     s.face_list = c.take<uint32_t>(R); s.keys = c.take<uint64_t>(R);
@@ -174,8 +177,15 @@
     if (!create) return nullptr;
     void* p = nullptr;
     if (hipHostMalloc(&p, 64, hipHostMallocCoherent | hipHostMallocPortable) != hipSuccess) return nullptr;
-    *reinterpret_cast<volatile uint32_t*>(p) = 0u;
+    memset(p, 0, 64);
     return g_overflow[dev] = reinterpret_cast<uint32_t*>(p);
+}
+uint32_t* timeout_word(uint32_t* overflow) { return overflow ? overflow + 1 : nullptr; }
+int check_timeout(uint32_t* overflow) {
+    volatile uint32_t* t = timeout_word(overflow);
+    if (!t || *t == 0u) return 0;
+    *t = 0u;
+    return fail("a bounded wait inside the tile scan + scatter launch timed out; the results of that call are invalid");
 }
 
 bool stream_is_capturing(hipStream_t st) {
@@ -221,14 +231,21 @@
     int dev = 0;
     DMR_HIP(hipGetDevice(&dev));
     uint32_t* overflow = overflow_word(dev, !async);
-
-    auto front = [&](unsigned long long* host_R, uint32_t host_seq, uint64_t capacity, uint32_t* ovf) -> int {
-        dmr::launch_project_verts(*s, ps.vproj, is.mats, is.tile_count, (size_t)(is.scan_tmp + dmr::SCAN_TMP_BUCKETS - is.tile_count), st);
+    if (check_timeout(overflow)) return 1;
+
+    const bool fusable = d.ntiles <= dmr::FUSE_MAX_TILES && timeout_word(overflow) != nullptr;
+    auto front = [&](bool scan, unsigned long long* host_R, uint32_t host_seq, uint64_t capacity, uint32_t* ovf) -> int {
+        dmr::launch_project_verts(*s, ps.vproj, is.mats, is.tile_count, counters_words(is, d.ntiles), st);
         dmr::launch_setup_faces(*s, tet, ps.vproj, d.gx, d.gy, d.r0, d.r1, fs.rect, fs.key_depth, fs.max_depth,
                                 fs.tiles_touched, is.tile_count, st);
-        dmr::launch_scan_tiles(d.ntiles, is.tile_count, is.tile_offset, is.tile_cursor, is.num_rendered, host_R, host_seq, is.tile_order,
-                               is.scan_tmp, (uint32_t)std::min<uint64_t>(capacity, 0xffffffffu), ovf, st);
+        if (scan)
+            dmr::launch_scan_tiles(d.ntiles, is.tile_count, is.tile_offset, is.num_rendered, host_R, host_seq, is.tile_order,
+                                   is.scan_tmp, (uint32_t)std::min<uint64_t>(capacity, 0xffffffffu), ovf, st);
         return 0;
+    };
+    auto fused = [&](unsigned long long* host_R, uint32_t host_seq, uint64_t capacity, uint32_t* ovf) {
+        return dmr::FusedScan{d.ntiles, is.tile_count, is.num_rendered, host_R, host_seq, is.tile_order,
+                              (uint32_t)std::min<uint64_t>(capacity, 0xffffffffu), ovf, is.fuse_sync, timeout_word(overflow)};
     };
     size_t seq_steps = 0;
     if (tet) {
@@ -250,7 +267,7 @@
             }
         }
     }
-    auto rest = [&](uint64_t capacity) -> int {
+    auto rest = [&](uint64_t capacity, const dmr::FusedScan* scan) -> int {
         BinningState tb, bs;
         const size_t mask_tiles = tet ? 0 : (size_t)d.ntiles;
         void* bb = alloc(ctx, DMR_BUF_BINNING, carve_binning(nullptr, (size_t)capacity, mask_tiles, (size_t)d.ntiles, seq_steps, tb));
@@ -258,8 +275,8 @@
         carve_binning(bb, (size_t)capacity, mask_tiles, (size_t)d.ntiles, seq_steps, bs);
 
         if (capacity > 0) {
-            dmr::launch_scatter_faces(*s, d.gx, d.gy, fs.rect, fs.key_depth, fs.tiles_touched, is.tile_cursor, bs.keys,
-                                      (uint32_t)capacity, tet ? nullptr : is.mask_offset, bs.mask_offset, bs.mask_first, st);
+            dmr::launch_scatter_faces(*s, d.gx, d.gy, fs.rect, fs.key_depth, fs.tiles_touched, is.tile_offset, is.tile_cursor, bs.keys,
+                                      (uint32_t)capacity, tet ? nullptr : is.mask_offset, bs.mask_offset, bs.mask_first, scan, st);
             if (d.ntiles > dmr::SCAN_SINGLE_MAX)
                 dmr::launch_sort_tiles(d.ntiles, is.tile_offset, is.tile_order, bs.keys, bs.face_list, bs.capacity, st);
         }
@@ -278,7 +295,8 @@
         if (!guess || !overflow)
             return fail("asynchronous / captured call without a size estimate: run one default (waiting) call with the same "
                         "view configuration first");
-        if (front(nullptr, 0u, guess, overflow) || rest(guess)) return 1;
+        const dmr::FusedScan fs_async = fused(nullptr, 0u, guess, overflow);
+        if (front(!fusable, nullptr, 0u, guess, overflow) || rest(guess, fusable ? &fs_async : nullptr)) return 1;
         *num_rendered = (int)guess;
         DMR_HIP(hipGetLastError());
         return 0;
@@ -286,19 +304,24 @@
     SizeRead* sr = size_read();
     if (!sr) return fail("hipHostMalloc failed");
     const uint32_t seq = sr->next_seq();
-    if (front(const_cast<unsigned long long*>(sr->word(0)), seq, ~0ull, nullptr)) return 1;
-    if (guess && rest(guess)) return 1;
+    unsigned long long* host_R = const_cast<unsigned long long*>(sr->word(0));
+    const bool fuse = guess && fusable;
+    const dmr::FusedScan fs_wait = fused(host_R, seq, ~0ull, nullptr);
+    if (front(!fuse, host_R, seq, ~0ull, nullptr)) return 1;
+    if (guess && rest(guess, fuse ? &fs_wait : nullptr)) return 1;
     unsigned long long R64 = 0;
     if (wait_size(sr->word(0), seq, st, &R64)) return 1;
+    if (check_timeout(overflow)) return 1;
     if (R64 > 0x7fffffffull) return fail("num_rendered overflows 31 bits");
     const int R = (int)R64;
     *num_rendered = R;
     if (!guess) {
-        if (rest((uint64_t)R)) return 1;
+        if (rest((uint64_t)R, nullptr)) return 1;
     } else if ((uint64_t)R > guess) {
         g_redo_count.fetch_add(1, std::memory_order_relaxed);
         DMR_HIP(hipStreamSynchronize(st));
-        if (front(nullptr, 0u, ~0ull, nullptr) || rest((uint64_t)R)) return 1;
+        if (check_timeout(overflow)) return 1;
+        if (front(true, nullptr, 0u, ~0ull, nullptr) || rest((uint64_t)R, nullptr)) return 1;
     }
     {
         std::lock_guard<std::mutex> lk(g_size_mu);
@@ -382,8 +405,8 @@
     uint32_t* w = overflow_word(dev, false);
     if (!w) return 0;
     volatile uint32_t* v = w;
-    const int r = *v != 0u;
-    if (reset) *v = 0u;
+    const int r = v[0] != 0u || v[1] != 0u;
+    if (reset) { v[0] = 0u; v[1] = 0u; }
     return r;
 }
 uint64_t dmr_redo_count(void) { return g_redo_count.load(std::memory_order_relaxed); }
diff --git a/dmesh_renderer_amd/csrc/dmr_binning.hip b/dmesh_renderer_amd/csrc/dmr_binning.hip
--- a/dmesh_renderer_amd/csrc/dmr_binning.hip
+++ b/dmesh_renderer_amd/csrc/dmr_binning.hip
@@ -176,90 +176,6 @@
     }
 }
 
-template <int FPT>
-__global__ void __launch_bounds__(256)
-k_scatter_faces_lds(int B, int F, int gx, int gy, const uint2* __restrict__ face_rect,
-                    const float* __restrict__ key_depth, const uint32_t* __restrict__ tiles_touched,
-                    uint32_t* __restrict__ tile_cursor, uint64_t* __restrict__ keys, uint32_t capacity,
-                    unsigned long long* __restrict__ mask_offset_dst, unsigned long long mask_offset, unsigned long long mask_first) {
-    if (mask_offset_dst && blockIdx.x == 0 && threadIdx.x == 0) { mask_offset_dst[0] = mask_offset; mask_offset_dst[1] = mask_first; }
-    __shared__ uint32_t s_hist[LDS_HIST_MAX];
-    __shared__ int s_box[4];
-    __shared__ BigFace s_big[BIG_MAX];
-    __shared__ uint32_t s_nbig;
-    const int tid = threadIdx.x;
-    if (tid == 0) s_nbig = 0u;
-    const int64_t BF = (int64_t)B * F;
-    const int64_t base = (int64_t)blockIdx.x * (256 * FPT);
-    const int view = (int)(base / F);
-    uint2 rr[FPT];
-    uint32_t touched[FPT];
-    bool mine[FPT];
-#pragma unroll
-    for (int it = 0; it < FPT; it++) {
-        const int64_t idx = base + it * 256 + tid;
-        touched[it] = idx < BF ? tiles_touched[idx] : 0u;
-        rr[it] = touched[it] ? face_rect[idx] : make_uint2(0, 0);
-        mine[it] = idx < BF && (int)(idx / F) == view;
-    }
-    const BinWindow w = bin_window<FPT>(s_box, view, rr, touched, mine, tid);
-    const int nw = w.wx * w.wy;
-    for (int t = tid; t < nw; t += 256) s_hist[t] = 0u;
-    __syncthreads();
-#pragma unroll
-    for (int it = 0; it < FPT; it++) {
-        if (!(w.lds && mine[it]) || touched[it] == 0 || touched[it] > BIG_RECT) continue;
-        const uint32_t minx = rr[it].x & 0xffffu, miny = rr[it].x >> 16, maxx = rr[it].y & 0xffffu, maxy = rr[it].y >> 16;
-        for (uint32_t y = miny; y < maxy; y++)
-            for (uint32_t x = minx; x < maxx; x++) atomicAdd(&s_hist[(y - w.y0) * w.wx + (x - w.x0)], 1u);
-    }
-    __syncthreads();
-    for (int y = tid / 64; y < w.wy; y += 4)
-        for (int x = tid % 64; x < w.wx; x += 64) {
-            const uint32_t c = s_hist[y * w.wx + x];
-            if (c) s_hist[y * w.wx + x] = atomicAdd(&tile_cursor[(uint32_t)view * gx * gy + (uint32_t)(w.y0 + y) * gx + (uint32_t)(w.x0 + x)], c);
-        }
-    __syncthreads();
-#pragma unroll
-    for (int it = 0; it < FPT; it++) {
-        if (touched[it] == 0) continue;
-        const int64_t idx = base + it * 256 + tid;
-        const int f = (int)(idx % F);
-        const uint32_t tb = (uint32_t)(idx / F) * gx * gy;
-        const uint32_t minx = rr[it].x & 0xffffu, miny = rr[it].x >> 16, maxx = rr[it].y & 0xffffu, maxy = rr[it].y >> 16;
-        const uint64_t key = ((uint64_t)__float_as_uint(key_depth[idx]) << 32) | (uint32_t)f;
-        if (touched[it] > BIG_RECT) {
-            const uint32_t q = atomicAdd(&s_nbig, 1u);
-            if (q < (uint32_t)BIG_MAX) { s_big[q] = BigFace{rr[it].x, rr[it].y, tb, (uint32_t)key, (uint32_t)(key >> 32)}; continue; }
-        }
-        const bool direct = !(w.lds && mine[it]) || touched[it] > BIG_RECT;
-        for (uint32_t y = miny; y < maxy; y++)
-            for (uint32_t x = minx; x < maxx; x++) {
-                const uint32_t slot = direct ? atomicAdd(&tile_cursor[tb + y * gx + x], 1u)
-                                             : atomicAdd(&s_hist[(y - w.y0) * w.wx + (x - w.x0)], 1u);
-                if (slot < capacity) keys[slot] = key;
-            }
-    }
-    __syncthreads();
-    const uint32_t nbig = min(s_nbig, (uint32_t)BIG_MAX);
-    for (uint32_t q = 0; q < nbig; q++) {
-        const BigFace f = s_big[q];
-        const uint64_t key = ((uint64_t)f.key_hi << 32) | f.key_lo;
-        for (RectWalk t(f.rect_lo & 0xffffu, f.rect_lo >> 16, f.rect_hi & 0xffffu, f.rect_hi >> 16, (uint32_t)tid); t.valid();) {
-            uint32_t tile[4], slot[4];
-#pragma unroll
-            for (int u = 0; u < 4; u++) {
-                tile[u] = 0xffffffffu;
-                if (t.valid()) { tile[u] = f.tile_base + t.y * gx + t.x; t.next(); }
-            }
-#pragma unroll
-            for (int u = 0; u < 4; u++) slot[u] = tile[u] != 0xffffffffu ? atomicAdd(&tile_cursor[tile[u]], 1u) : 0xffffffffu;
-#pragma unroll
-            for (int u = 0; u < 4; u++) if (slot[u] < capacity) keys[slot[u]] = key;
-        }
-    }
-}
-
 constexpr int ORDER_BUCKETS = 64;
 __device__ __forceinline__ int order_bucket(uint32_t n) { return ORDER_BUCKETS - 1 - (int)min(n >> 4, (uint32_t)(ORDER_BUCKETS - 1)); }
 constexpr int ORDER_COPIES = 16;
@@ -314,7 +230,7 @@
 
 __global__ void __launch_bounds__(1024)
 k_scan_tiles(int n, const uint32_t* __restrict__ tile_count, uint32_t* __restrict__ tile_offset,
-             uint32_t* __restrict__ tile_cursor, int* __restrict__ num_rendered, unsigned long long* __restrict__ host_num_rendered,
+             int* __restrict__ num_rendered, unsigned long long* __restrict__ host_num_rendered,
              uint32_t host_seq, uint32_t* __restrict__ tile_order, uint32_t capacity, uint32_t* __restrict__ overflow) {
     static_assert(ORDER_CELLS == 1024, "one counter cell per thread");
     __shared__ uint32_t wave_sum[17];
@@ -342,7 +258,7 @@
 #pragma unroll
     for (int j = 0; j < SCAN_BATCH; j++) {
         const int i = j * 1024 + tid;
-        if (i < n) { const uint32_t o = slab[i]; tile_offset[i] = o; tile_cursor[i] = o; }
+        if (i < n) tile_offset[i] = slab[i];
     }
     __syncthreads();
 #pragma unroll
@@ -441,7 +357,7 @@
 template <bool ORDER>
 __global__ void __launch_bounds__(1024)
 k_scan_tiles_final(int n, const uint32_t* __restrict__ tile_count, const uint32_t* __restrict__ len_offset, const uint32_t* __restrict__ blk_sum,
-                   uint32_t* __restrict__ bucket_cursor, uint32_t* __restrict__ tile_offset, uint32_t* __restrict__ tile_cursor,
+                   uint32_t* __restrict__ bucket_cursor, uint32_t* __restrict__ tile_offset, uint32_t* __restrict__ tile_used,
                    uint32_t* __restrict__ tile_order) {
     __shared__ uint32_t wave_sum[17];
     __shared__ uint32_t bucket[ORDER_CELLS + 1];
@@ -456,7 +372,7 @@
         c[j] = begin + j < end ? tile_count[begin + j] : 0u;
         if (!ORDER && begin + j < end) {
             c[j] = record_bound(c[j], len_offset[begin + j + 1] - len_offset[begin + j]);
-            tile_cursor[begin + j] = 0u;
+            tile_used[begin + j] = 0u;
         }
     }
 #pragma unroll
@@ -486,7 +402,7 @@
 #pragma unroll
     for (int j = 0; j < SCAN_BATCH; j++) {
         const bool in = begin + j < end;
-        if (in) { tile_offset[begin + j] = run; if (ORDER) tile_cursor[begin + j] = run; }
+        if (in) tile_offset[begin + j] = run;
         run += c[j];
         if (!ORDER) continue;
         const bool empty = in && c[j] == 0u;
@@ -535,6 +451,292 @@
         hit_offset[n] = wave_sum[16]; *hit_total = s_total;
         if (host_hit_total) *host_hit_total = host_size_word(host_seq, s_total);
         if (overflow && s_total > (unsigned long long)capacity) *overflow = 1u;
+    }
+}
+
+constexpr int FUSE_VALS = ORDER_BUCKETS + 2;
+constexpr int SYNC_TICKET = 0, SYNC_DONE = 1, SYNC_CURSOR = 4, SYNC_GRANULES = 128;
+static_assert(SYNC_CURSOR + ORDER_BUCKETS + 1 <= SYNC_GRANULES, "bucket cursors in front of the granules");
+static_assert(FUSE_CHUNK == 256 * SCAN_BATCH, "a chunk is 8 tiles per thread of a 256-thread workgroup");
+static_assert(ORDER_CELLS == ORDER_BUCKETS * ORDER_COPIES, "the empty-tile cell follows the last bucket's copies");
+constexpr uint32_t FUSE_SPIN_MAX = 1u << 20;
+size_t fuse_sync_words(int ntiles) { return SYNC_GRANULES + 2 * (size_t)FUSE_VALS * (size_t)((ntiles + FUSE_CHUNK - 1) / FUSE_CHUNK); }
+
+typedef __attribute__((address_space(1))) uint32_t gu32;
+typedef __attribute__((address_space(1))) unsigned long long gu64;
+
+constexpr int FL_CELLS = 0;
+constexpr int FL_PREF = 1040;
+constexpr int FL_OWN = FL_PREF + 80;
+constexpr int FL_WAVE = FL_OWN + 80;
+constexpr int FL_WORDS = FL_WAVE + 17;
+static_assert(FL_PREF >= ORDER_CELLS + 1 && FL_WORDS <= LDS_HIST_MAX, "chunk LDS layout");
+
+__device__ __forceinline__ void fused_timeout(const FusedScan& a) { *reinterpret_cast<volatile uint32_t*>(a.timeout) = 1u; }
+
+__device__ __forceinline__ void chunk_load(const uint32_t* __restrict__ tile_count, int n, int begin, uint32_t (&c)[SCAN_BATCH]) {
+    if (begin + SCAN_BATCH <= n) {
+        const uint4 lo = *reinterpret_cast<const uint4*>(tile_count + begin), hi = *reinterpret_cast<const uint4*>(tile_count + begin + 4);
+        c[0] = lo.x; c[1] = lo.y; c[2] = lo.z; c[3] = lo.w; c[4] = hi.x; c[5] = hi.y; c[6] = hi.z; c[7] = hi.w;
+    } else {
+#pragma unroll
+        for (int j = 0; j < SCAN_BATCH; j++) c[j] = begin + j < n ? tile_count[begin + j] : 0u;
+    }
+}
+__device__ __forceinline__ void chunk_cells(uint32_t* cells, int n, int begin, const uint32_t (&c)[SCAN_BATCH], int lane) {
+    int n_empty = 0;
+#pragma unroll
+    for (int j = 0; j < SCAN_BATCH; j++) {
+        if (begin + j >= n) continue;
+        if (c[j]) atomicAdd(&cells[order_cell(c[j], lane)], 1u);
+        else n_empty++;
+    }
+#pragma unroll
+    for (int d = 32; d > 0; d >>= 1) n_empty += __shfl_xor(n_empty, d, 64);
+    if (lane == 0 && n_empty) atomicAdd(&cells[ORDER_CELLS], (uint32_t)n_empty);
+}
+
+__device__ __forceinline__ bool fused_wait_done(const FusedScan& a, int nchunks, uint32_t* s_flag, int tid) {
+    if (tid == 0) {
+        uint32_t ok = 1u;
+        for (uint32_t spins = 0; __hip_atomic_load((gu32*)(a.sync + SYNC_DONE), __ATOMIC_RELAXED, __HIP_MEMORY_SCOPE_AGENT) < (uint32_t)nchunks; spins++) {
+            if (spins == FUSE_SPIN_MAX) { fused_timeout(a); ok = 0u; break; }
+            __builtin_amdgcn_s_sleep(2);
+        }
+        __builtin_amdgcn_fence(__ATOMIC_ACQUIRE, "agent");
+        asm volatile("s_waitcnt vmcnt(0)" ::: "memory");
+        *s_flag = ok;
+    }
+    __syncthreads();
+    return *s_flag != 0u;
+}
+
+__device__ __forceinline__ void fused_publish_done(const FusedScan& a, int tid) {
+    asm volatile("s_waitcnt vmcnt(0)" ::: "memory");
+    __syncthreads();
+    if (tid == 0) {
+        __builtin_amdgcn_fence(__ATOMIC_RELEASE, "agent");
+        asm volatile("s_waitcnt vmcnt(0)" ::: "memory");
+        __hip_atomic_fetch_add((gu32*)(a.sync + SYNC_DONE), 1u, __ATOMIC_RELAXED, __HIP_MEMORY_SCOPE_AGENT);
+    }
+}
+
+__device__ void fused_scan_chunk(const FusedScan& a, uint32_t* tile_offset, int chunk, int nchunks, uint32_t* lds, int tid) {
+    const int lane = tid & 63, n = a.ntiles;
+    uint32_t* cells = lds + FL_CELLS; uint32_t* pref = lds + FL_PREF; uint32_t* own = lds + FL_OWN; uint32_t* wave_sum = lds + FL_WAVE;
+    for (int i = tid; i < FL_WORDS; i += 256) lds[i] = 0u;
+    const int begin = chunk * FUSE_CHUNK + tid * SCAN_BATCH;
+    uint32_t c[SCAN_BATCH], local = 0;
+    chunk_load(a.tile_count, n, begin, c);
+    __syncthreads();
+    chunk_cells(cells, n, begin, c, lane);
+#pragma unroll
+    for (int j = 0; j < SCAN_BATCH; j++) local += c[j];
+    const uint32_t run = block_exclusive_scan(local, tid, wave_sum);
+    gu64* g = (gu64*)(a.sync + SYNC_GRANULES);
+    if (tid < FUSE_VALS) {
+        uint32_t v = 0;
+        if (tid == 0) v = wave_sum[16];
+        else if (tid <= ORDER_BUCKETS) {
+#pragma unroll
+            for (int q = 0; q < ORDER_COPIES; q++) v += cells[(tid - 1) * ORDER_COPIES + q];
+        } else v = cells[ORDER_CELLS];
+        own[tid] = v;
+        __hip_atomic_store(g + (size_t)chunk * FUSE_VALS + tid, (1ull << 32) | v, __ATOMIC_RELAXED, __HIP_MEMORY_SCOPE_AGENT);
+    }
+    constexpr int LB = 4;
+    const int items = chunk * FUSE_VALS;
+    for (int i0 = 0; i0 < items; i0 += 256 * LB) {
+        unsigned long long x[LB];
+        for (uint32_t spins = 0;; spins++) {
+            bool ready = true;
+#pragma unroll
+            for (int k = 0; k < LB; k++) x[k] = __hip_atomic_load(g + min(i0 + tid + 256 * k, items - 1), __ATOMIC_RELAXED, __HIP_MEMORY_SCOPE_AGENT);
+#pragma unroll
+            for (int k = 0; k < LB; k++) ready &= (x[k] >> 32) != 0ull;
+            if (ready) break;
+            if (spins == FUSE_SPIN_MAX) { fused_timeout(a); break; }
+            __builtin_amdgcn_s_sleep(1);
+        }
+#pragma unroll
+        for (int k = 0; k < LB; k++) {
+            const int i = i0 + tid + 256 * k;
+            if (i < items) atomicAdd(&pref[i % FUSE_VALS], (uint32_t)x[k]);
+        }
+    }
+    __syncthreads();
+    uint32_t o[SCAN_BATCH], r = pref[0] + run;
+#pragma unroll
+    for (int j = 0; j < SCAN_BATCH; j++) { o[j] = r; r += c[j]; }
+    if (begin + SCAN_BATCH <= n) {
+        *reinterpret_cast<uint4*>(tile_offset + begin) = make_uint4(o[0], o[1], o[2], o[3]);
+        *reinterpret_cast<uint4*>(tile_offset + begin + 4) = make_uint4(o[4], o[5], o[6], o[7]);
+    } else {
+#pragma unroll
+        for (int j = 0; j < SCAN_BATCH; j++) if (begin + j < n) tile_offset[begin + j] = o[j];
+    }
+    if (chunk == nchunks - 1) {
+        if (tid < 64) {
+            const uint32_t t = pref[1 + tid] + own[1 + tid];
+            uint32_t incl = t;
+#pragma unroll
+            for (int d = 1; d < 64; d <<= 1) {
+                const uint32_t u = __shfl_up(incl, d, 64);
+                if (lane >= d) incl += u;
+            }
+            static_assert(ORDER_BUCKETS == 64, "one lane per bucket");
+            __hip_atomic_store((gu32*)(a.sync + SYNC_CURSOR + tid), incl - t, __ATOMIC_RELAXED, __HIP_MEMORY_SCOPE_AGENT);
+            if (tid == 63) __hip_atomic_store((gu32*)(a.sync + SYNC_CURSOR + ORDER_BUCKETS), incl, __ATOMIC_RELAXED, __HIP_MEMORY_SCOPE_AGENT);
+        }
+        if (tid == 0) {
+            const uint32_t total = pref[0] + own[0];
+            tile_offset[n] = total; *a.num_rendered = (int)total;
+            if (a.host_num_rendered) *a.host_num_rendered = host_size_word(a.host_seq, total);
+            if (a.overflow && total > a.capacity) *a.overflow = 1u;
+        }
+    }
+    fused_publish_done(a, tid);
+}
+
+__device__ void fused_order_chunk(const FusedScan& a, uint32_t* __restrict__ tile_order, int chunk, int nchunks, uint32_t* lds,
+                                  uint32_t* s_flag, int tid) {
+    const int lane = tid & 63, n = a.ntiles;
+    uint32_t* cells = lds + FL_CELLS;
+    for (int i = tid; i <= ORDER_CELLS; i += 256) cells[i] = 0u;
+    const int begin = chunk * FUSE_CHUNK + tid * SCAN_BATCH;
+    uint32_t c[SCAN_BATCH];
+    chunk_load(a.tile_count, n, begin, c);
+    __syncthreads();
+    chunk_cells(cells, n, begin, c, lane);
+    if (!fused_wait_done(a, nchunks, s_flag, tid)) return;
+    if (tid <= ORDER_BUCKETS) {
+        uint32_t* cl = cells + tid * ORDER_COPIES;
+        const int ncl = tid < ORDER_BUCKETS ? ORDER_COPIES : 1;
+        uint32_t cnt = 0;
+        for (int q = 0; q < ncl; q++) cnt += cl[q];
+        uint32_t b = cnt ? __hip_atomic_fetch_add((gu32*)(a.sync + SYNC_CURSOR + tid), cnt, __ATOMIC_RELAXED, __HIP_MEMORY_SCOPE_AGENT) : 0u;
+        for (int q = 0; q < ncl; q++) { const uint32_t k = cl[q]; cl[q] = b; b += k; }
+    }
+    __syncthreads();
+#pragma unroll
+    for (int j = 0; j < SCAN_BATCH; j++) {
+        const bool in = begin + j < n;
+        const bool empty = in && c[j] == 0u;
+        const uint64_t em = __ballot(empty);
+        uint32_t ebase = 0;
+        if (em) {
+            const int leader = __ffsll((long long)em) - 1;
+            if (lane == leader) ebase = atomicAdd(&cells[ORDER_CELLS], (uint32_t)__popcll(em));
+            ebase = __shfl(ebase, leader, 64);
+        }
+        uint32_t pos = 0xffffffffu;
+        if (empty) pos = ebase + (uint32_t)__popcll(em & ((1ull << lane) - 1ull));
+        else if (in) pos = atomicAdd(&cells[order_cell(c[j], lane)], 1u);
+        if (pos < (uint32_t)n) tile_order[pos] = (uint32_t)(begin + j);
+    }
+}
+
+constexpr uint32_t RESERVED = 0x80000000u;
+
+template <int FPT>
+__global__ void __launch_bounds__(256)
+k_scatter_faces_lds(int B, int F, int gx, int gy, const uint2* __restrict__ face_rect,
+                    const float* __restrict__ key_depth, const uint32_t* __restrict__ tiles_touched,
+                    uint32_t* tile_offset, uint32_t* __restrict__ tile_cursor, uint64_t* __restrict__ keys, uint32_t capacity,
+                    unsigned long long* __restrict__ mask_offset_dst, unsigned long long mask_offset, unsigned long long mask_first,
+                    FusedScan scan, int nchunks, int nface_blocks) {
+    if (mask_offset_dst && blockIdx.x == 0 && threadIdx.x == 0) { mask_offset_dst[0] = mask_offset; mask_offset_dst[1] = mask_first; }
+    __shared__ __attribute__((aligned(16))) uint32_t s_hist[LDS_HIST_MAX];
+    __shared__ int s_box[4];
+    __shared__ BigFace s_big[BIG_MAX];
+    __shared__ uint32_t s_nbig, s_ticket, s_flag;
+    const int tid = threadIdx.x;
+    int blk = (int)blockIdx.x;
+    if (nchunks) {
+        if (tid == 0) s_ticket = __hip_atomic_fetch_add((gu32*)(scan.sync + SYNC_TICKET), 1u, __ATOMIC_RELAXED, __HIP_MEMORY_SCOPE_AGENT);
+        __syncthreads();
+        blk = (int)s_ticket;
+        if (blk < nchunks) { fused_scan_chunk(scan, tile_offset, blk, nchunks, s_hist, tid); return; }
+        blk -= nchunks;
+        if (blk >= nface_blocks) { fused_order_chunk(scan, scan.tile_order, blk - nface_blocks, nchunks, s_hist, &s_flag, tid); return; }
+    }
+    if (tid == 0) s_nbig = 0u;
+    const int64_t BF = (int64_t)B * F;
+    const int64_t base = (int64_t)blk * (256 * FPT);
+    const int view = (int)(base / F);
+    uint2 rr[FPT];
+    uint32_t touched[FPT];
+    bool mine[FPT];
+#pragma unroll
+    for (int it = 0; it < FPT; it++) {
+        const int64_t idx = base + it * 256 + tid;
+        touched[it] = idx < BF ? tiles_touched[idx] : 0u;
+        rr[it] = touched[it] ? face_rect[idx] : make_uint2(0, 0);
+        mine[it] = idx < BF && (int)(idx / F) == view;
+    }
+    const BinWindow w = bin_window<FPT>(s_box, view, rr, touched, mine, tid);
+    const int nw = w.wx * w.wy;
+    for (int t = tid; t < nw; t += 256) s_hist[t] = 0u;
+    __syncthreads();
+#pragma unroll
+    for (int it = 0; it < FPT; it++) {
+        if (!(w.lds && mine[it]) || touched[it] == 0 || touched[it] > BIG_RECT) continue;
+        const uint32_t minx = rr[it].x & 0xffffu, miny = rr[it].x >> 16, maxx = rr[it].y & 0xffffu, maxy = rr[it].y >> 16;
+        for (uint32_t y = miny; y < maxy; y++)
+            for (uint32_t x = minx; x < maxx; x++) atomicAdd(&s_hist[(y - w.y0) * w.wx + (x - w.x0)], 1u);
+    }
+    __syncthreads();
+    for (int y = tid / 64; y < w.wy; y += 4)
+        for (int x = tid % 64; x < w.wx; x += 64) {
+            const uint32_t c = s_hist[y * w.wx + x];
+            if (c) s_hist[y * w.wx + x] = RESERVED | atomicAdd(&tile_cursor[(uint32_t)view * gx * gy + (uint32_t)(w.y0 + y) * gx + (uint32_t)(w.x0 + x)], c);
+        }
+    __syncthreads();
+    if (nchunks && !fused_wait_done(scan, nchunks, &s_flag, tid)) return;
+    for (int y = tid / 64; y < w.wy; y += 4)
+        for (int x = tid % 64; x < w.wx; x += 64) {
+            const uint32_t r = s_hist[y * w.wx + x];
+            if (r & RESERVED) s_hist[y * w.wx + x] = tile_offset[(uint32_t)view * gx * gy + (uint32_t)(w.y0 + y) * gx + (uint32_t)(w.x0 + x)] + (r & ~RESERVED);
+        }
+    __syncthreads();
+#pragma unroll
+    for (int it = 0; it < FPT; it++) {
+        if (touched[it] == 0) continue;
+        const int64_t idx = base + it * 256 + tid;
+        const int f = (int)(idx % F);
+        const uint32_t tb = (uint32_t)(idx / F) * gx * gy;
+        const uint32_t minx = rr[it].x & 0xffffu, miny = rr[it].x >> 16, maxx = rr[it].y & 0xffffu, maxy = rr[it].y >> 16;
+        const uint64_t key = ((uint64_t)__float_as_uint(key_depth[idx]) << 32) | (uint32_t)f;
+        if (touched[it] > BIG_RECT) {
+            const uint32_t q = atomicAdd(&s_nbig, 1u);
+            if (q < (uint32_t)BIG_MAX) { s_big[q] = BigFace{rr[it].x, rr[it].y, tb, (uint32_t)key, (uint32_t)(key >> 32)}; continue; }
+        }
+        const bool direct = !(w.lds && mine[it]) || touched[it] > BIG_RECT;
+        for (uint32_t y = miny; y < maxy; y++)
+            for (uint32_t x = minx; x < maxx; x++) {
+                const uint32_t t = tb + y * gx + x;
+                const uint32_t slot = direct ? tile_offset[t] + atomicAdd(&tile_cursor[t], 1u)
+                                             : atomicAdd(&s_hist[(y - w.y0) * w.wx + (x - w.x0)], 1u);
+                if (slot < capacity) keys[slot] = key;
+            }
+    }
+    __syncthreads();
+    const uint32_t nbig = min(s_nbig, (uint32_t)BIG_MAX);
+    for (uint32_t q = 0; q < nbig; q++) {
+        const BigFace f = s_big[q];
+        const uint64_t key = ((uint64_t)f.key_hi << 32) | f.key_lo;
+        for (RectWalk t(f.rect_lo & 0xffffu, f.rect_lo >> 16, f.rect_hi & 0xffffu, f.rect_hi >> 16, (uint32_t)tid); t.valid();) {
+            uint32_t tile[4], slot[4];
+#pragma unroll
+            for (int u = 0; u < 4; u++) {
+                tile[u] = 0xffffffffu;
+                if (t.valid()) { tile[u] = f.tile_base + t.y * gx + t.x; t.next(); }
+            }
+#pragma unroll
+            for (int u = 0; u < 4; u++) slot[u] = tile[u] != 0xffffffffu ? tile_offset[tile[u]] + atomicAdd(&tile_cursor[tile[u]], 1u) : 0xffffffffu;
+#pragma unroll
+            for (int u = 0; u < 4; u++) if (tile[u] != 0xffffffffu && slot[u] < capacity) keys[slot[u]] = key;
+        }
     }
 }
 
@@ -576,12 +778,12 @@
 #undef DMR_SETUP
 }
 
-void launch_scan_tiles(int ntiles, const uint32_t* tile_count, uint32_t* tile_offset, uint32_t* tile_cursor,
+void launch_scan_tiles(int ntiles, const uint32_t* tile_count, uint32_t* tile_offset,
                        int* num_rendered, unsigned long long* host_num_rendered, uint32_t host_seq, uint32_t* tile_order, uint32_t* scan_tmp,
                        uint32_t capacity, uint32_t* overflow, hipStream_t st) {
     StageScope t(DMR_STAGE_SCAN, st);
     if (ntiles <= SCAN_SINGLE_MAX) {
-        k_scan_tiles<<<dim3(1), dim3(1024), 0, st>>>(ntiles, tile_count, tile_offset, tile_cursor, num_rendered, host_num_rendered, host_seq, tile_order,
+        k_scan_tiles<<<dim3(1), dim3(1024), 0, st>>>(ntiles, tile_count, tile_offset, num_rendered, host_num_rendered, host_seq, tile_order,
                                                     capacity, overflow);
         return;
     }
@@ -591,7 +793,7 @@
     k_scan_tiles_partial<true><<<dim3(nblk), dim3(1024), 0, st>>>(ntiles, tile_count, nullptr, blk_sum, bucket);
     k_scan_tiles_blocks<<<dim3(1), dim3(1024), 0, st>>>(nblk, ntiles, blk_sum, bucket, tile_offset, num_rendered, host_num_rendered,
                                                         nullptr, nullptr, host_seq, capacity, overflow);
-    k_scan_tiles_final<true><<<dim3(nblk), dim3(1024), 0, st>>>(ntiles, tile_count, nullptr, blk_sum, bucket, tile_offset, tile_cursor, tile_order);
+    k_scan_tiles_final<true><<<dim3(nblk), dim3(1024), 0, st>>>(ntiles, tile_count, nullptr, blk_sum, bucket, tile_offset, nullptr, tile_order);
 }
 
 size_t scan_tmp_words(int ntiles) { return SCAN_TMP_BUCKETS + (size_t)(ntiles + SCAN_BLOCK_TILES - 1) / SCAN_BLOCK_TILES + 1; }
@@ -613,15 +815,20 @@
 }
 
 void launch_scatter_faces(const dmr_scene& s, int gx, int gy, const uint2* face_rect, const float* key_depth,
-                          const uint32_t* tiles_touched, uint32_t* tile_cursor, uint64_t* keys, uint32_t capacity,
-                          unsigned long long* mask_offset_dst, unsigned long long mask_offset, unsigned long long mask_first, hipStream_t st) {
+                          const uint32_t* tiles_touched, uint32_t* tile_offset, uint32_t* tile_cursor, uint64_t* keys, uint32_t capacity,
+                          unsigned long long* mask_offset_dst, unsigned long long mask_offset, unsigned long long mask_first,
+                          const FusedScan* scan, hipStream_t st) {
     const int64_t n = (int64_t)s.B * s.F;
-    if (n == 0) return;
+    const int nchunks = scan ? (scan->ntiles + FUSE_CHUNK - 1) / FUSE_CHUNK : 0;
+    if (n == 0 && nchunks == 0) return;
     StageScope t(DMR_STAGE_SCATTER, st);
     const int fpt = bin_fpt(n);
-    const dim3 grid((unsigned)((n + 256 * fpt - 1) / (256 * fpt))), block(256);
+    const int nfb = (int)((n + 256 * fpt - 1) / (256 * fpt));
+    const FusedScan fs = scan ? *scan : FusedScan{};
+    const dim3 grid((unsigned)(nfb + 2 * nchunks)), block(256);
 #define DMR_SCATTER(FPT) k_scatter_faces_lds<FPT><<<grid, block, 0, st>>>(s.B, s.F, gx, gy, face_rect, key_depth, tiles_touched, \
-                                                                         tile_cursor, keys, capacity, mask_offset_dst, mask_offset, mask_first)
+                                                                         tile_offset, tile_cursor, keys, capacity, mask_offset_dst, mask_offset, mask_first, \
+                                                                         fs, nchunks, nfb)
     if (fpt == 1) DMR_SCATTER(1); else if (fpt == 2) DMR_SCATTER(2); else DMR_SCATTER(4);
 #undef DMR_SCATTER
 }
diff --git a/dmesh_renderer_amd/csrc/dmr_kernels.hpp b/dmesh_renderer_amd/csrc/dmr_kernels.hpp
--- a/dmesh_renderer_amd/csrc/dmr_kernels.hpp
+++ b/dmesh_renderer_amd/csrc/dmr_kernels.hpp
@@ -39,12 +39,23 @@
 __host__ __device__ inline unsigned long long host_size_word(uint32_t seq, unsigned long long size) {
     return ((unsigned long long)(seq & 0xffffffu) << 40) | (size < (1ull << 40) ? size : (1ull << 40) - 1ull);
 }
-void launch_scan_tiles(int ntiles, const uint32_t* tile_count, uint32_t* tile_offset, uint32_t* tile_cursor,
+void launch_scan_tiles(int ntiles, const uint32_t* tile_count, uint32_t* tile_offset,
                        int* num_rendered, unsigned long long* host_num_rendered, uint32_t host_seq, uint32_t* tile_order, uint32_t* scan_tmp,
                        uint32_t capacity, uint32_t* overflow, hipStream_t st);
+constexpr int FUSE_CHUNK = 2048;
+constexpr int FUSE_MAX_CHUNKS = 64;
+constexpr int FUSE_MAX_TILES = FUSE_CHUNK * FUSE_MAX_CHUNKS;
+size_t fuse_sync_words(int ntiles);
+struct FusedScan {
+    int ntiles; const uint32_t* tile_count;
+    int* num_rendered; unsigned long long* host_num_rendered; uint32_t host_seq;
+    uint32_t* tile_order; uint32_t capacity; uint32_t* overflow;
+    uint32_t* sync; uint32_t* timeout;
+};
 void launch_scatter_faces(const dmr_scene& s, int gx, int gy, const uint2* face_rect, const float* key_depth,
-                          const uint32_t* tiles_touched, uint32_t* tile_cursor, uint64_t* keys, uint32_t capacity,
-                          unsigned long long* mask_offset_dst, unsigned long long mask_offset, unsigned long long mask_first, hipStream_t st);
+                          const uint32_t* tiles_touched, uint32_t* tile_offset, uint32_t* tile_cursor, uint64_t* keys, uint32_t capacity,
+                          unsigned long long* mask_offset_dst, unsigned long long mask_offset, unsigned long long mask_first,
+                          const FusedScan* scan, hipStream_t st);
 void launch_sort_tiles(int ntiles, const uint32_t* tile_offset, const uint32_t* tile_order, uint64_t* keys,
                        uint32_t* face_list, uint32_t capacity, hipStream_t st);
 
```

Result: slower. 6951, median of 6 (-2.3%).
